# onesamblack/distributed-torch-horovod-gcp

Hardware: NVIDIA H100
Metric: images/sec (whole job, device-timed, max over ranks) ResNet-50 synthetic ImageNet training (higher is better)
Workload: dtype bf16

## Files before the change

distributed_torch_horovod_gcp_b200/csrc/conv_sm90.cu:

```cuda
#include <cuda.h>
#include <cuda_bf16.h>
#include <cuda_runtime.h>
#include <limits.h>
#include <stdint.h>
#include <stdio.h>
#include <stdlib.h>
#include <string.h>

#include "sm90_common.cuh"

namespace {

constexpr int MAX_TAPS = 9;
constexpr int MAX_CLASSES = 4;

struct ConvTap {
  int amap;
  int dw, dh;
  int wcol;
};
struct ConvClass {
  int ntaps;
  int out_map;
  ConvTap taps[MAX_TAPS];
};
struct ConvParams {
  GemmParams g;
  int num_classes;
  int kc_per_tap;
  int bw, bh, bn;
  int sw, sh;
  int tiles_w, tiles_h, tiles_n;
  int num_taps_total;
  int out_w, out_h, out_n;
  ConvClass cls[MAX_CLASSES];
};
struct alignas(64) ConvMaps {
  CUtensorMap a[4];
  CUtensorMap b;
  CUtensorMap out[4];
};

enum { MODE_FPROP = 0, MODE_DGRAD = 1, MODE_WGRAD = 2 };

template <int BN, int MODE>
struct ConvWork {
  static constexpr bool kStats = MODE == MODE_FPROP, kSplitK = MODE == MODE_WGRAD;
  static constexpr bool B_MN = MODE != MODE_FPROP;
  const ConvMaps& maps;
  const ConvParams& p;
  int nnb, pix_tiles, tiles, items, kb_per_split;

  __device__ ConvWork(const ConvMaps& maps_, const ConvParams& p_)
      : maps(maps_), p(p_), nnb(p_.g.num_n_blocks), pix_tiles(p_.tiles_w * p_.tiles_h * p_.tiles_n),
        tiles(MODE == MODE_WGRAD ? p_.g.num_m_blocks * nnb * p_.num_taps_total : p_.num_classes * pix_tiles * nnb),
        items(tiles * p_.g.splits),
        kb_per_split(MODE == MODE_WGRAD ? (pix_tiles + p_.g.splits - 1) / p_.g.splits : 0) {}
  __device__ void prefetch() const {
    for (int i = 0; i < 4; ++i) tma_prefetch_desc(&maps.a[i]);
    tma_prefetch_desc(&maps.b);
    for (int i = 0; i < 4; ++i) tma_prefetch_desc(&maps.out[i]);
  }
  __device__ int num_kb(int w) const {
    if (MODE != MODE_WGRAD) return p.cls[(w / nnb) / pix_tiles].ntaps * p.kc_per_tap;
    const int kb0 = (w / tiles) * kb_per_split;
    return min(kb0 + kb_per_split, pix_tiles) - kb0;
  }
  template <class Next>
  __device__ void load(int w, Next& next) const {
    if (MODE != MODE_WGRAD) {
      const int nt = w % nnb;
      const int rest = w / nnb;
      const int mt = rest % pix_tiles;
      const ConvClass& cl = p.cls[rest / pix_tiles];
      const int w0 = (mt % p.tiles_w) * p.bw;
      const int h0 = ((mt / p.tiles_w) % p.tiles_h) * p.bh;
      const int n0 = (mt / (p.tiles_w * p.tiles_h)) * p.bn;
      const int n_idx = nt * BN;
      for (int t = 0; t < cl.ntaps; ++t) {
        const ConvTap tap = cl.taps[t];
        for (int kc = 0; kc < p.kc_per_tap; ++kc) {
          const Stage s = next();
          tma_load_4d(&maps.a[tap.amap], s.bar, s.a, kc * BLOCK_K, w0 + tap.dw, h0 + tap.dh, n0);
          if (!B_MN) {
            tma_load_2d(&maps.b, s.bar, s.b, tap.wcol + kc * BLOCK_K, n_idx);
          } else {
#pragma unroll
            for (int c = 0; c < BN / 64; ++c)
              tma_load_2d(&maps.b, s.bar, s.b + c * (BLOCK_K * 128), tap.wcol + n_idx + 64 * c, kc * BLOCK_K);
          }
        }
      }
    } else {
      const int tile = w % tiles, split = w / tiles;
      const ConvTap tap = p.cls[0].taps[tile % p.num_taps_total];
      const int mn = tile / p.num_taps_total;
      const int m_idx = (mn / nnb) * BLOCK_M;
      const int n_idx = (mn % nnb) * BN;
      const int kb0 = split * kb_per_split;
      const int kb1 = min(kb0 + kb_per_split, pix_tiles);
      for (int kb = kb0; kb < kb1; ++kb) {
        const int w0 = (kb % p.tiles_w) * p.bw;
        const int h0 = ((kb / p.tiles_w) % p.tiles_h) * p.bh;
        const int n0 = (kb / (p.tiles_w * p.tiles_h)) * p.bn;
        const Stage s = next();
#pragma unroll
        for (int c = 0; c < BLOCK_M / 64; ++c)
          tma_load_4d(&maps.out[0], s.bar, s.a + c * (BLOCK_K * 128), m_idx + 64 * c, w0, h0, n0);
#pragma unroll
        for (int c = 0; c < BN / 64; ++c)
          tma_load_4d(&maps.a[tap.amap], s.bar, s.b + c * (BLOCK_K * 128), n_idx + 64 * c, w0 + tap.dw,
                      h0 + tap.dh, n0);
      }
    }
  }
  __device__ Slab slab(int w, int q) const {
    if (MODE != MODE_WGRAD) {
      const int nt = w % nnb;
      const int rest = w / nnb;
      const int mt = rest % pix_tiles;
      const int r0 = q * 32;
      StoreAt at;
      at.rank4 = 1;
      at.w = (mt % p.tiles_w) * p.bw + (r0 % p.bw);
      at.h = ((mt / p.tiles_w) % p.tiles_h) * p.bh + (r0 / p.bw) % p.bh;
      at.n = (mt / (p.tiles_w * p.tiles_h)) * p.bn + r0 / (p.bw * p.bh);
      at.c_ptr = nullptr;
      at.sw = p.sw; at.sh = p.sh;
      at.vw = p.out_w - at.w; at.vh = p.out_h - at.h; at.vn = p.out_n - at.n;
      return Slab{&maps.out[p.cls[rest / pix_tiles].out_map], nullptr, 0, nt * BN, at, 0, 0, 0};
    }
    const int tile = w % tiles;
    const ConvTap tap = p.cls[0].taps[tile % p.num_taps_total];
    const int mn = tile / p.num_taps_total;
    const int m_idx = (mn / nnb) * BLOCK_M;
    float* c_ptr = (p.g.splits > 1 ? p.g.splitk_ws + (long long)(w / tiles) * p.g.splitk_slice
                                   : reinterpret_cast<float*>(p.g.C)) + tap.wcol;
    return Slab{nullptr, nullptr, m_idx + q * 32, (mn % nnb) * BN, StoreAt{0, 0, 0, 0, c_ptr, 32, 1, 32, 1, 1},
                tile, m_idx, tap.wcol};
  }
};

template <int BN, int MODE>
__global__ void __launch_bounds__(NUM_THREADS, 1)
conv_bf16_kernel(const __grid_constant__ ConvMaps maps, const __grid_constant__ ConvParams p) {
  persistent_body<BN, MODE == MODE_WGRAD, MODE != MODE_FPROP>(ConvWork<BN, MODE>(maps, p), p.g);
}

int make_map4(CUtensorMap* m, const void* ptr, uint64_t C, uint64_t Wd, uint64_t Hd, uint64_t Nd, uint64_t pw,
              uint64_t ph, uint64_t pn, uint32_t bw, uint32_t bh, uint32_t bn) {
  const cuuint64_t dims[4] = {C, Wd, Hd, Nd};
  const cuuint64_t strides[3] = {pw * 2, ph * 2, pn * 2};
  const cuuint32_t box[4] = {64, bw, bh, bn};
  return encode_map(m, ptr, 4, dims, strides, box);
}

void choose_box(int W, int H, int N, int rows, int* bw, int* bh, int* bn) {
  double best = 1e30;
  *bw = 1; *bh = 1; *bn = rows;
  for (int w = 1; w <= rows; w <<= 1) {
    for (int h = 1; w * h <= rows; h <<= 1) {
      const int n = rows / (w * h);
      const double covered = (double)((W + w - 1) / w * w) * ((H + h - 1) / h * h) * ((N + n - 1) / n * n);
      const double score = covered - 1e-3 * w - 1e-6 * h;
      if (score < best) { best = score; *bw = w; *bh = h; *bn = n; }
    }
  }
}

int floordiv2(int e) { return (e >= 0) ? e / 2 : -((-e + 1) / 2); }

struct ConvShape {
  int N, H, W, Cin, Cout, R, S, stride, pad, OH, OW;
};

int check_shape(ConvShape& s) {
  if (s.R != s.S || (s.R != 1 && s.R != 3)) return fail("only 1x1 and 3x3 filters");
  if (s.pad != (s.R - 1) / 2) return fail("padding must be (R-1)/2");
  if (s.stride != 1 && s.stride != 2) return fail("stride must be 1 or 2");
  if (s.stride == 2 && ((s.H | s.W) & 1)) return fail("stride 2 needs even H and W");
  if ((s.Cin % 8) || (s.Cout % 8)) return fail("channels must be multiples of 8");
  s.OH = s.H / s.stride;
  s.OW = s.W / s.stride;
  return 0;
}

int make_parity_maps(CUtensorMap* maps, const void* base, int C, int W, int H, int N, int bw, int bh, int bn) {
  for (int ph = 0; ph < 2; ++ph)
    for (int pw = 0; pw < 2; ++pw) {
      const __nv_bfloat16* ptr = reinterpret_cast<const __nv_bfloat16*>(base) + ((size_t)ph * W + pw) * C;
      if (make_map4(&maps[ph * 2 + pw], ptr, C, W / 2, H / 2, N, 2 * (uint64_t)C, 2 * (uint64_t)W * C,
                    (uint64_t)H * W * C, bw, bh, bn))
        return -1;
    }
  return 0;
}

void forward_taps(ConvClass& cl, int R, int S, int Cin, int stride, int pad) {
  for (int r = 0; r < R; ++r)
    for (int c = 0; c < S; ++c) {
      ConvTap& t = cl.taps[cl.ntaps++];
      const int eh = r - pad, ew = c - pad;
      if (stride == 1) {
        t.amap = 0; t.dh = eh; t.dw = ew;
      } else {
        const int ph = eh & 1, pw = ew & 1;
        t.amap = ph * 2 + pw; t.dh = floordiv2(eh - ph); t.dw = floordiv2(ew - pw);
      }
      t.wcol = (r * S + c) * Cin;
    }
}

void slab_box(ConvParams& p) {
  p.sw = p.bw < 32 ? p.bw : 32;
  p.sh = (32 / p.sw) < p.bh ? (32 / p.sw) : p.bh;
}

template <int MODE>
int launch_conv(const ConvMaps& maps, const ConvParams& p, int BN, int work, int max_ctas, cudaStream_t st) {
  if (BN == 64) return launch_persistent<conv_bf16_kernel<64, MODE>, 64>(work, max_ctas, st, maps, p);
  return launch_persistent<conv_bf16_kernel<128, MODE>, 128>(work, max_ctas, st, maps, p);
}

ConvParams conv_params() {
  ConvParams p;
  memset(&p, 0, sizeof(p));
  p.g.M = INT_MAX;
  p.g.splits = 1;
  p.g.alpha = 1.0f;
  return p;
}

}

extern "C" {

const char* b200dp_conv_last_error() { return g_err; }

int b200dp_conv_fprop(const void* x, const void* w, void* y, int N, int H, int W, int Cin, int Cout, int R, int S,
                      int stride, int pad, int block_n, int max_ctas, float* stats, unsigned long long stream) {
  if (ensure_init()) return -1;
  ConvShape s{N, H, W, Cin, Cout, R, S, stride, pad, 0, 0};
  if (check_shape(s)) return -1;
  if (((uintptr_t)x | (uintptr_t)w | (uintptr_t)y) & 15) return fail("pointers must be 16-byte aligned");
  const int BN = pick_bn(Cout, block_n);
  if (BN < 0) return -1;
  ConvMaps maps;
  ConvParams p = conv_params();
  p.g.N = Cout; p.g.ldc = Cout; p.g.C = y; p.g.out_mode = 0;
  p.g.stats = stats;
  if (stats != nullptr && Cout > STATS_MAX_N) return fail("stats: Cout <= 2048 required");
  p.g.num_n_blocks = (Cout + BN - 1) / BN;
  p.g.num_k_blocks = (Cin + BLOCK_K - 1) / BLOCK_K;
  p.kc_per_tap = p.g.num_k_blocks;
  choose_box(s.OW, s.OH, N, BLOCK_M, &p.bw, &p.bh, &p.bn);
  p.tiles_w = (s.OW + p.bw - 1) / p.bw; p.tiles_h = (s.OH + p.bh - 1) / p.bh; p.tiles_n = (N + p.bn - 1) / p.bn;
  p.num_classes = 1;
  p.num_taps_total = R * S;
  p.out_w = s.OW; p.out_h = s.OH; p.out_n = N;
  forward_taps(p.cls[0], R, S, Cin, stride, pad);
  if (stride == 1) {
    if (make_map4(&maps.a[0], x, Cin, W, H, N, Cin, (uint64_t)W * Cin, (uint64_t)H * W * Cin, p.bw, p.bh, p.bn))
      return -1;
    maps.a[1] = maps.a[2] = maps.a[3] = maps.a[0];
  } else if (make_parity_maps(maps.a, x, Cin, W, H, N, p.bw, p.bh, p.bn)) {
    return -1;
  }
  if (make_map2(&maps.b, w, Cout, (uint64_t)R * S * Cin, (uint64_t)R * S * Cin, BN)) return -1;
  slab_box(p);
  if (make_map4(&maps.out[0], y, Cout, s.OW, s.OH, N, Cout, (uint64_t)s.OW * Cout, (uint64_t)s.OH * s.OW * Cout, p.sw,
                p.sh, 32 / (p.sw * p.sh)))
    return -1;
  maps.out[1] = maps.out[2] = maps.out[3] = maps.out[0];
  const int work = p.tiles_w * p.tiles_h * p.tiles_n * p.g.num_n_blocks;
  return launch_conv<MODE_FPROP>(maps, p, BN, work, max_ctas, (cudaStream_t)(uintptr_t)stream);
}

int b200dp_conv_dgrad(const void* dy, const void* w, void* dx, int N, int H, int W, int Cin, int Cout, int R, int S,
                      int stride, int pad, int block_n, int max_ctas, unsigned long long stream) {
  if (ensure_init()) return -1;
  ConvShape s{N, H, W, Cin, Cout, R, S, stride, pad, 0, 0};
  if (check_shape(s)) return -1;
  if (((uintptr_t)dy | (uintptr_t)w | (uintptr_t)dx) & 15) return fail("pointers must be 16-byte aligned");
  cudaStream_t st = (cudaStream_t)(uintptr_t)stream;
  const int BN = pick_bn(Cin, block_n);
  if (BN < 0) return -1;
  ConvMaps maps;
  ConvParams p = conv_params();
  p.g.N = Cin; p.g.ldc = Cin; p.g.C = dx; p.g.out_mode = 0;
  p.g.num_n_blocks = (Cin + BN - 1) / BN;
  p.g.num_k_blocks = (Cout + BLOCK_K - 1) / BLOCK_K;
  p.kc_per_tap = p.g.num_k_blocks;
  choose_box(s.OW, s.OH, N, BLOCK_M, &p.bw, &p.bh, &p.bn);
  p.tiles_w = (s.OW + p.bw - 1) / p.bw; p.tiles_h = (s.OH + p.bh - 1) / p.bh; p.tiles_n = (N + p.bn - 1) / p.bn;
  p.num_taps_total = R * S;
  p.out_w = s.OW; p.out_h = s.OH; p.out_n = N;
  slab_box(p);
  const int sn = 32 / (p.sw * p.sh);
  if (make_map4(&maps.a[0], dy, Cout, s.OW, s.OH, N, Cout, (uint64_t)s.OW * Cout, (uint64_t)s.OH * s.OW * Cout,
                p.bw, p.bh, p.bn))
    return -1;
  maps.a[1] = maps.a[2] = maps.a[3] = maps.a[0];
  if (make_map2(&maps.b, w, Cout, (uint64_t)R * S * Cin, (uint64_t)R * S * Cin, 64)) return -1;
  if (stride == 1) {
    p.num_classes = 1;
    ConvClass& cl = p.cls[0];
    cl.out_map = 0;
    for (int r = 0; r < R; ++r)
      for (int c = 0; c < S; ++c) {
        ConvTap& t = cl.taps[cl.ntaps++];
        t.amap = 0; t.dh = pad - r; t.dw = pad - c; t.wcol = (r * S + c) * Cin;
      }
    if (make_map4(&maps.out[0], dx, Cin, W, H, N, Cin, (uint64_t)W * Cin, (uint64_t)H * W * Cin, p.sw, p.sh, sn))
      return -1;
    maps.out[1] = maps.out[2] = maps.out[3] = maps.out[0];
  } else {
    if (make_parity_maps(maps.out, dx, Cin, W, H, N, p.sw, p.sh, sn)) return -1;
    bool any_empty = false;
    for (int ph = 0; ph < 2; ++ph)
      for (int pw = 0; pw < 2; ++pw) {
        ConvClass cl;
        memset(&cl, 0, sizeof(cl));
        cl.out_map = ph * 2 + pw;
        for (int r = 0; r < R; ++r) {
          if ((ph + pad - r) & 1) continue;
          for (int c = 0; c < S; ++c) {
            if ((pw + pad - c) & 1) continue;
            ConvTap& t = cl.taps[cl.ntaps++];
            t.amap = 0; t.dh = floordiv2(ph + pad - r); t.dw = floordiv2(pw + pad - c); t.wcol = (r * S + c) * Cin;
          }
        }
        if (cl.ntaps == 0) { any_empty = true; continue; }
        p.cls[p.num_classes++] = cl;
      }
    if (any_empty) {
      cudaError_t e = cudaMemsetAsync(dx, 0, (size_t)N * H * W * Cin * 2, st);
      if (e != cudaSuccess) return fail(cudaGetErrorString(e), (int)e);
    }
  }
  const int work = p.num_classes * p.tiles_w * p.tiles_h * p.tiles_n * p.g.num_n_blocks;
  return launch_conv<MODE_DGRAD>(maps, p, BN, work, max_ctas, st);
}

int b200dp_conv_wgrad(const void* dy, const void* x, void* dw_acc, int N, int H, int W, int Cin, int Cout, int R,
                      int S, int stride, int pad, int splits, int block_n, int max_ctas, unsigned long long stream) {
  if (ensure_init()) return -1;
  ConvShape s{N, H, W, Cin, Cout, R, S, stride, pad, 0, 0};
  if (check_shape(s)) return -1;
  if (((uintptr_t)dy | (uintptr_t)x | (uintptr_t)dw_acc) & 15) return fail("pointers must be 16-byte aligned");
  const int BN = pick_bn(Cin, block_n);
  if (BN < 0) return -1;
  ConvMaps maps;
  ConvParams p = conv_params();
  p.g.M = Cout; p.g.N = Cin; p.g.ldc = R * S * Cin; p.g.C = dw_acc; p.g.out_mode = 1;
  p.g.num_m_blocks = (Cout + BLOCK_M - 1) / BLOCK_M;
  p.g.num_n_blocks = (Cin + BN - 1) / BN;
  choose_box(s.OW, s.OH, N, BLOCK_K, &p.bw, &p.bh, &p.bn);
  p.tiles_w = (s.OW + p.bw - 1) / p.bw; p.tiles_h = (s.OH + p.bh - 1) / p.bh; p.tiles_n = (N + p.bn - 1) / p.bn;
  const int kblocks = p.tiles_w * p.tiles_h * p.tiles_n;
  p.num_classes = 1;
  p.num_taps_total = R * S;
  forward_taps(p.cls[0], R, S, Cin, stride, pad);
  const int tiles = p.g.num_m_blocks * p.g.num_n_blocks * R * S;
  if (splits <= 0) {
    splits = g_num_sms / tiles;
    if (splits < 1) splits = 1;
    const int max_splits = kblocks / 8 > 1 ? kblocks / 8 : 1;
    if (splits > max_splits) splits = max_splits;
  }
  p.g.splits = normalize_splits(splits, kblocks);
  if (stride == 1) {
    if (make_map4(&maps.a[0], x, Cin, W, H, N, Cin, (uint64_t)W * Cin, (uint64_t)H * W * Cin, p.bw, p.bh, p.bn))
      return -1;
    maps.a[1] = maps.a[2] = maps.a[3] = maps.a[0];
  } else if (make_parity_maps(maps.a, x, Cin, W, H, N, p.bw, p.bh, p.bn)) {
    return -1;
  }
  if (make_map4(&maps.out[0], dy, Cout, s.OW, s.OH, N, Cout, (uint64_t)s.OW * Cout, (uint64_t)s.OH * s.OW * Cout,
                p.bw, p.bh, p.bn))
    return -1;
  maps.out[1] = maps.out[2] = maps.out[3] = maps.out[0];
  maps.b = maps.out[0];
  cudaStream_t st = (cudaStream_t)(uintptr_t)stream;
  if (p.g.splits > 1) p.g.splitk_slice = (long long)Cout * p.g.ldc;
  return run_splitk(p.g, tiles, st,
                    [&] { return launch_conv<MODE_WGRAD>(maps, p, BN, tiles * p.g.splits, max_ctas, st); });
}

}
```

distributed_torch_horovod_gcp_b200/csrc/gemm_sm90.cu:

```cuda
#include <cuda.h>
#include <cuda_bf16.h>
#include <cuda_runtime.h>
#include <stdint.h>

#include "sm90_common.cuh"

namespace {

template <int BN, bool A_MN, bool B_MN>
struct GemmWork {
  static constexpr bool kStats = true, kSplitK = true;
  const CUtensorMap *a, *b, *c, *z;
  const GemmParams& p;
  int tiles, items, kb_per_split;

  __device__ GemmWork(const CUtensorMap* a_, const CUtensorMap* b_, const CUtensorMap* c_, const CUtensorMap* z_,
                      const GemmParams& p_)
      : a(a_), b(b_), c(c_), z(z_), p(p_), tiles(p_.num_m_blocks * p_.num_n_blocks), items(tiles * p_.splits),
        kb_per_split((p_.num_k_blocks + p_.splits - 1) / p_.splits) {}
  __device__ void prefetch() const {
    tma_prefetch_desc(a);
    tma_prefetch_desc(b);
    if (p.out_mode == 0) tma_prefetch_desc(c);
    if (p.out_mode == 0 && p.preact != nullptr) tma_prefetch_desc(z);
  }
  __device__ int m_idx(int tile) const {
    return (p.n_fastest ? tile / p.num_n_blocks : tile % p.num_m_blocks) * BLOCK_M;
  }
  __device__ int n_idx(int tile) const { return (p.n_fastest ? tile % p.num_n_blocks : tile / p.num_m_blocks) * BN; }
  __device__ int num_kb(int w) const {
    const int kb0 = (w / tiles) * kb_per_split;
    return min(kb0 + kb_per_split, p.num_k_blocks) - kb0;
  }
  template <class Next>
  __device__ void load(int w, Next& next) const {
    const int tile = w % tiles;
    const int m0 = m_idx(tile), n0 = n_idx(tile);
    const int kb0 = (w / tiles) * kb_per_split;
    const int kb1 = min(kb0 + kb_per_split, p.num_k_blocks);
    for (int kb = kb0; kb < kb1; ++kb) {
      const Stage s = next();
      const int k_idx = kb * BLOCK_K;
      if (!A_MN) {
        tma_load_2d(a, s.bar, s.a, k_idx, m0);
      } else {
#pragma unroll
        for (int c = 0; c < BLOCK_M / 64; ++c)
          tma_load_2d(a, s.bar, s.a + c * (BLOCK_K * 128), m0 + 64 * c, k_idx);
      }
      if (!B_MN) {
        tma_load_2d(b, s.bar, s.b, k_idx, n0);
      } else {
#pragma unroll
        for (int c = 0; c < BN / 64; ++c)
          tma_load_2d(b, s.bar, s.b + c * (BLOCK_K * 128), n0 + 64 * c, k_idx);
      }
    }
  }
  __device__ Slab slab(int w, int q) const {
    const int tile = w % tiles, split = w / tiles;
    const int m0 = m_idx(tile);
    return Slab{c, z, m0 + q * 32, n_idx(tile),
                StoreAt{0, 0, 0, 0, p.splits > 1 ? p.splitk_ws + (long long)split * p.splitk_slice : nullptr},
                tile, m0, 0};
  }
};

template <int BN, bool A_MN, bool B_MN>
__global__ void __launch_bounds__(NUM_THREADS, 1)
gemm_bf16_kernel(const __grid_constant__ CUtensorMap map_a, const __grid_constant__ CUtensorMap map_b,
                 const __grid_constant__ CUtensorMap map_c, const __grid_constant__ CUtensorMap map_z,
                 const __grid_constant__ GemmParams p) {
  persistent_body<BN, A_MN, B_MN>(GemmWork<BN, A_MN, B_MN>(&map_a, &map_b, &map_c, &map_z, p), p);
}

int launch_bn(int BN, int a_mn, int b_mn, const CUtensorMap& ma, const CUtensorMap& mb, const CUtensorMap& mc,
              const CUtensorMap& mz, const GemmParams& p, int max_ctas, cudaStream_t st) {
  const int work = p.num_m_blocks * p.num_n_blocks * p.splits;
#define LAUNCH(BNV, AMN, BMN) \
  launch_persistent<gemm_bf16_kernel<BNV, AMN, BMN>, BNV>(work, max_ctas, st, ma, mb, mc, mz, p)
#define DISPATCH(BNV)                                          \
  if (BN == BNV) {                                             \
    if (!a_mn && !b_mn) return LAUNCH(BNV, false, false);      \
    if (!a_mn && b_mn) return LAUNCH(BNV, false, true);        \
    if (a_mn && !b_mn) return LAUNCH(BNV, true, false);        \
    return LAUNCH(BNV, true, true);                            \
  }
  DISPATCH(64)
  DISPATCH(128)
#undef DISPATCH
#undef LAUNCH
  return fail("unreachable");
}

}

extern "C" {

const char* b200dp_gemm_last_error() { return g_err; }

int b200dp_gemm_bf16(const void* A, const void* B, void* C, int M, int N, int K, int lda, int ldb, int ldc,
                     int a_mn, int b_mn, const void* bias_bf16, const void* bias_f32, const void* residual,
                     void* preact, int act, int out_mode, float alpha, int splits, int block_n, int max_ctas,
                     float* stats, const void* res_mask, unsigned long long stream) {
  if (ensure_init()) return -1;
  if (M <= 0 || N <= 0 || K <= 0) return fail("bad shape");
  if ((N % 8) || (lda % 8) || (ldb % 8) || (ldc % 4) || ((out_mode == 0) && (ldc % 8)))
    return fail("alignment: N, lda, ldb, ldc must be multiples of 8");
  if (((uintptr_t)A | (uintptr_t)B | (uintptr_t)C) & 15) return fail("pointers must be 16-byte aligned");
  const int BN = pick_bn(N, block_n);
  if (BN < 0) return -1;
  GemmParams p{};
  p.M = M; p.N = N; p.ldc = ldc;
  p.num_m_blocks = (M + BLOCK_M - 1) / BLOCK_M;
  p.num_n_blocks = (N + BN - 1) / BN;
  p.num_k_blocks = (K + BLOCK_K - 1) / BLOCK_K;
  p.splits = normalize_splits(splits, p.num_k_blocks);
  if (p.splits > 1 && out_mode != 1) return fail("split-K requires out_mode=1 (fp32 accumulate)");
  p.act = act; p.out_mode = out_mode; p.C = C; p.bias = bias_bf16; p.bias_f32 = bias_f32;
  p.residual = residual; p.preact = preact; p.alpha = alpha;
  p.stats = stats;
  p.res_mask = reinterpret_cast<const unsigned char*>(res_mask);
  if (res_mask != nullptr && (residual == nullptr || preact != nullptr || act > 2 || out_mode != 0 || (N % 64) ||
                              ldc != N))
    return fail("res_mask: plain bf16 residual, dense rows and N % 64 == 0 required");
  if (stats != nullptr && (N > STATS_MAX_N || out_mode != 0)) return fail("stats: N <= 2048 and bf16 output required");
  p.n_fastest = ((size_t)N * (size_t)K * 2 <= ((size_t)20 << 20)) ? 1 : 0;
  CUtensorMap ma, mb, mc, mz;
  if (a_mn ? make_map2(&ma, A, K, M, lda, BLOCK_K) : make_map2(&ma, A, M, K, lda, BLOCK_M)) return -1;
  if (b_mn ? make_map2(&mb, B, K, N, ldb, BLOCK_K) : make_map2(&mb, B, N, K, ldb, BN)) return -1;
  if (out_mode == 0) {
    if (make_map2(&mc, C, M, N, ldc, 32)) return -1;
  } else {
    mc = ma;
  }
  if (out_mode == 0 && preact != nullptr) {
    if (make_map2(&mz, preact, M, N, ldc, 32)) return -1;
  } else {
    mz = mc;
  }
  cudaStream_t st = (cudaStream_t)(uintptr_t)stream;
  if (p.splits > 1) p.splitk_slice = (long long)M * ldc;
  return run_splitk(p, p.num_m_blocks * p.num_n_blocks, st,
                    [&] { return launch_bn(BN, a_mn, b_mn, ma, mb, mc, mz, p, max_ctas, st); });
}

}
```

distributed_torch_horovod_gcp_b200/csrc/sm90_common.cuh:

```cuda
#pragma once
#include <cuda.h>
#include <cuda_bf16.h>
#include <cuda_runtime.h>
#include <stdint.h>
#include <stdio.h>

namespace {

constexpr int BLOCK_M = 128;
constexpr int BLOCK_K = 64;
constexpr int WGMMA_K = 16;
constexpr int NUM_THREADS = 384;
constexpr int EPI_WARPS = 8;
constexpr int SMEM_LIMIT = 232448;

struct GemmParams {
  int M, N;
  int ldc;
  int num_m_blocks, num_n_blocks, num_k_blocks;
  int splits;
  int act;
  int out_mode;
  void* C;
  const void* bias;
  const void* bias_f32;
  const void* residual;
  void* preact;
  int n_fastest;
  float alpha;
  const unsigned char* res_mask;
  float* stats;
  float* splitk_ws;
  int* splitk_count;
  long long splitk_slice;
};

constexpr int STATS_MAX_N = 2048;
constexpr int STATS_WARP_FLOATS = 256;
constexpr int STATS_SMEM_BYTES = 8 * STATS_WARP_FLOATS * 4;

__device__ __forceinline__ uint32_t smem_u32(const void* p) {
  return static_cast<uint32_t>(__cvta_generic_to_shared(p));
}
__device__ __forceinline__ void mbar_init(uint64_t* bar, uint32_t count) {
  asm volatile("mbarrier.init.shared::cta.b64 [%0], %1;" ::"r"(smem_u32(bar)), "r"(count));
}
__device__ __forceinline__ void mbar_expect_tx(uint64_t* bar, uint32_t bytes) {
  asm volatile("mbarrier.arrive.expect_tx.shared::cta.b64 _, [%0], %1;" ::"r"(smem_u32(bar)),
               "r"(bytes)
               : "memory");
}
__device__ __forceinline__ void mbar_arrive(uint64_t* bar) {
  asm volatile("mbarrier.arrive.shared::cta.b64 _, [%0];" ::"r"(smem_u32(bar)) : "memory");
}
__device__ __forceinline__ void mbar_wait(uint64_t* bar, uint32_t parity) {
  uint32_t done = 0;
  unsigned long long t0 = 0;
  for (uint32_t tries = 0; !done; ++tries) {
    asm volatile(
        "{\n\t"
        ".reg .pred p;\n\t"
        "mbarrier.try_wait.parity.shared::cta.b64 p, [%1], %2;\n\t"
        "selp.u32 %0, 1, 0, p;\n\t"
        "}\n"
        : "=r"(done)
        : "r"(smem_u32(bar)), "r"(parity)
        : "memory");
    if (!done && (tries & 1023u) == 1023u) {
      unsigned long long now;
      asm volatile("mov.u64 %0, %%globaltimer;" : "=l"(now));
      if (t0 == 0) t0 = now;
      else if (now - t0 > 4000000000ull) __trap();
    }
  }
}
__device__ __forceinline__ void tma_load_2d(const CUtensorMap* map, uint64_t* bar, void* dst, int c0,
                                            int c1) {
  asm volatile(
      "cp.async.bulk.tensor.2d.shared::cluster.global.mbarrier::complete_tx::bytes [%0], [%1, {%3, %4}], "
      "[%2];" ::"r"(smem_u32(dst)),
      "l"(map), "r"(smem_u32(bar)), "r"(c0), "r"(c1)
      : "memory");
}
__device__ __forceinline__ void tma_store_2d(const CUtensorMap* map, const void* src, int c0, int c1) {
  asm volatile("cp.async.bulk.tensor.2d.global.shared::cta.bulk_group [%0, {%2, %3}], [%1];" ::"l"(map),
               "r"(smem_u32(src)), "r"(c0), "r"(c1)
               : "memory");
}
__device__ __forceinline__ void tma_load_4d(const CUtensorMap* map, uint64_t* bar, void* dst, int c0, int c1,
                                            int c2, int c3) {
  asm volatile(
      "cp.async.bulk.tensor.4d.shared::cluster.global.mbarrier::complete_tx::bytes [%0], "
      "[%1, {%3, %4, %5, %6}], [%2];" ::"r"(smem_u32(dst)),
      "l"(map), "r"(smem_u32(bar)), "r"(c0), "r"(c1), "r"(c2), "r"(c3)
      : "memory");
}
__device__ __forceinline__ void tma_store_4d(const CUtensorMap* map, const void* src, int c0, int c1, int c2,
                                             int c3) {
  asm volatile("cp.async.bulk.tensor.4d.global.shared::cta.bulk_group [%0, {%2, %3, %4, %5}], [%1];" ::"l"(map),
               "r"(smem_u32(src)), "r"(c0), "r"(c1), "r"(c2), "r"(c3)
               : "memory");
}
__device__ __forceinline__ void tma_store_commit() { asm volatile("cp.async.bulk.commit_group;" ::: "memory"); }
template <int N>
__device__ __forceinline__ void tma_store_wait_read() {
  asm volatile("cp.async.bulk.wait_group.read %0;" ::"n"(N) : "memory");
}
__device__ __forceinline__ void tma_store_wait_all() { asm volatile("cp.async.bulk.wait_group 0;" ::: "memory"); }
__device__ __forceinline__ void fence_async_smem() { asm volatile("fence.proxy.async.shared::cta;" ::: "memory"); }
__device__ __forceinline__ void tma_prefetch_desc(const CUtensorMap* map) {
  asm volatile("prefetch.tensormap [%0];" ::"l"(map) : "memory");
}
__device__ __forceinline__ void wg_fence() { asm volatile("wgmma.fence.sync.aligned;" ::: "memory"); }
__device__ __forceinline__ void wg_commit() { asm volatile("wgmma.commit_group.sync.aligned;" ::: "memory"); }
template <int N>
__device__ __forceinline__ void wg_wait() {
  asm volatile("wgmma.wait_group.sync.aligned %0;" ::"n"(N) : "memory");
}
template <int R>
__device__ __forceinline__ void wg_fence_operands(float* d) {
#pragma unroll
  for (int i = 0; i < R; ++i) asm volatile("" : "+f"(d[i])::"memory");
}
__device__ __forceinline__ void named_bar(int id, int count) {
  asm volatile("bar.sync %0, %1;" ::"r"(id), "r"(count) : "memory");
}

template <int TA, int TB>
__device__ __forceinline__ void wgmma_bf16_n64(float* d, uint64_t a, uint64_t b, uint32_t acc) {
  asm volatile(
      "{\n\t.reg .pred p;\n\tsetp.ne.b32 p, %34, 0;\n\t"
      "wgmma.mma_async.sync.aligned.m64n64k16.f32.bf16.bf16 {%0, %1, %2, %3, %4, %5, %6, %7, %8, %9, %10, %11, %12, %13, %14, %15, %16, %17, %18, %19, %20, %21, %22, %23, %24, %25, %26, %27, %28, %29, %30, %31}, %32, %33, p, 1, 1, %35, %36;\n\t}\n"
      : "+f"(d[0]), "+f"(d[1]), "+f"(d[2]), "+f"(d[3]), "+f"(d[4]), "+f"(d[5]), "+f"(d[6]), "+f"(d[7]), "+f"(d[8]), "+f"(d[9]), "+f"(d[10]), "+f"(d[11]), "+f"(d[12]), "+f"(d[13]), "+f"(d[14]), "+f"(d[15]), "+f"(d[16]), "+f"(d[17]), "+f"(d[18]), "+f"(d[19]), "+f"(d[20]), "+f"(d[21]), "+f"(d[22]), "+f"(d[23]), "+f"(d[24]), "+f"(d[25]), "+f"(d[26]), "+f"(d[27]), "+f"(d[28]), "+f"(d[29]), "+f"(d[30]), "+f"(d[31])
      : "l"(a), "l"(b), "r"(acc), "n"(TA), "n"(TB));
}

template <int TA, int TB>
__device__ __forceinline__ void wgmma_bf16_n128(float* d, uint64_t a, uint64_t b, uint32_t acc) {
  asm volatile(
      "{\n\t.reg .pred p;\n\tsetp.ne.b32 p, %66, 0;\n\t"
      "wgmma.mma_async.sync.aligned.m64n128k16.f32.bf16.bf16 {%0, %1, %2, %3, %4, %5, %6, %7, %8, %9, %10, %11, %12, %13, %14, %15, %16, %17, %18, %19, %20, %21, %22, %23, %24, %25, %26, %27, %28, %29, %30, %31, %32, %33, %34, %35, %36, %37, %38, %39, %40, %41, %42, %43, %44, %45, %46, %47, %48, %49, %50, %51, %52, %53, %54, %55, %56, %57, %58, %59, %60, %61, %62, %63}, %64, %65, p, 1, 1, %67, %68;\n\t}\n"
      : "+f"(d[0]), "+f"(d[1]), "+f"(d[2]), "+f"(d[3]), "+f"(d[4]), "+f"(d[5]), "+f"(d[6]), "+f"(d[7]), "+f"(d[8]), "+f"(d[9]), "+f"(d[10]), "+f"(d[11]), "+f"(d[12]), "+f"(d[13]), "+f"(d[14]), "+f"(d[15]), "+f"(d[16]), "+f"(d[17]), "+f"(d[18]), "+f"(d[19]), "+f"(d[20]), "+f"(d[21]), "+f"(d[22]), "+f"(d[23]), "+f"(d[24]), "+f"(d[25]), "+f"(d[26]), "+f"(d[27]), "+f"(d[28]), "+f"(d[29]), "+f"(d[30]), "+f"(d[31]), "+f"(d[32]), "+f"(d[33]), "+f"(d[34]), "+f"(d[35]), "+f"(d[36]), "+f"(d[37]), "+f"(d[38]), "+f"(d[39]), "+f"(d[40]), "+f"(d[41]), "+f"(d[42]), "+f"(d[43]), "+f"(d[44]), "+f"(d[45]), "+f"(d[46]), "+f"(d[47]), "+f"(d[48]), "+f"(d[49]), "+f"(d[50]), "+f"(d[51]), "+f"(d[52]), "+f"(d[53]), "+f"(d[54]), "+f"(d[55]), "+f"(d[56]), "+f"(d[57]), "+f"(d[58]), "+f"(d[59]), "+f"(d[60]), "+f"(d[61]), "+f"(d[62]), "+f"(d[63])
      : "l"(a), "l"(b), "r"(acc), "n"(TA), "n"(TB));
}

__device__ __forceinline__ void wgmma_tf32_n32(float* d, uint64_t a, uint64_t b, uint32_t acc) {
  asm volatile(
      "{\n\t.reg .pred p;\n\tsetp.ne.b32 p, %18, 0;\n\t"
      "wgmma.mma_async.sync.aligned.m64n32k8.f32.tf32.tf32 {%0, %1, %2, %3, %4, %5, %6, %7, %8, %9, %10, %11, %12, %13, %14, %15}, %16, %17, p, 1, 1;\n\t}\n"
      : "+f"(d[0]), "+f"(d[1]), "+f"(d[2]), "+f"(d[3]), "+f"(d[4]), "+f"(d[5]), "+f"(d[6]), "+f"(d[7]), "+f"(d[8]), "+f"(d[9]), "+f"(d[10]), "+f"(d[11]), "+f"(d[12]), "+f"(d[13]), "+f"(d[14]), "+f"(d[15])
      : "l"(a), "l"(b), "r"(acc));
}


template <int N>
__device__ __forceinline__ void acc_to_smem(const float* d, uint32_t img, int ld, int row0) {
  const int t = threadIdx.x & 127;
  const int r = row0 + (t >> 5) * 16 + ((t & 31) >> 2);
  const uint32_t p0 = img + (uint32_t)((r * ld + 2 * (t & 3)) * 4);
  const uint32_t p1 = p0 + (uint32_t)(8 * ld * 4);
#pragma unroll
  for (int j = 0; j < N / 8; ++j) {
    asm volatile("st.shared.v2.f32 [%0], {%1, %2};" ::"r"(p0 + j * 32), "f"(d[4 * j]), "f"(d[4 * j + 1]) : "memory");
    asm volatile("st.shared.v2.f32 [%0], {%1, %2};" ::"r"(p1 + j * 32), "f"(d[4 * j + 2]), "f"(d[4 * j + 3]) : "memory");
  }
}
__device__ __forceinline__ void acc_ld32(uint32_t addr, uint32_t* r) {
#pragma unroll
  for (int i = 0; i < 8; ++i)
    asm volatile("ld.shared.v4.b32 {%0, %1, %2, %3}, [%4];"
                 : "=r"(r[4 * i]), "=r"(r[4 * i + 1]), "=r"(r[4 * i + 2]), "=r"(r[4 * i + 3])
                 : "r"(addr + 16 * i)
                 : "memory");
}

__device__ __forceinline__ uint64_t make_desc(uint32_t smem_addr, uint32_t lbo_bytes,
                                              uint32_t sbo_bytes) {
  uint64_t d = 0;
  d |= (uint64_t)((smem_addr & 0x3FFFF) >> 4);
  d |= (uint64_t)((lbo_bytes >> 4) & 0x3FFF) << 16;
  d |= (uint64_t)((sbo_bytes >> 4) & 0x3FFF) << 32;
  d |= (uint64_t)1 << 62;
  return d;
}

__device__ __forceinline__ bool elect_one() {
  uint32_t pred;
  asm volatile(
      "{\n\t"
      ".reg .pred p;\n\t"
      "elect.sync _|p, 0xffffffff;\n\t"
      "selp.u32 %0, 1, 0, p;\n\t"
      "}\n"
      : "=r"(pred));
  return pred != 0;
}

__device__ __forceinline__ uint64_t make_desc_base(uint32_t lbo_bytes, uint32_t sbo_bytes) {
  return make_desc(0, lbo_bytes, sbo_bytes);
}
__device__ __forceinline__ uint64_t desc_addr(uint32_t smem_addr) { return (uint64_t)((smem_addr & 0x3FFFF) >> 4); }

template <int BN, bool TA, bool TB>
__device__ __forceinline__ void wgmma_bf16(float* d, uint64_t a, uint64_t b, uint32_t acc) {
  static_assert(BN == 64 || BN == 128, "wgmma width");
  if constexpr (BN == 64) wgmma_bf16_n64<TA ? 1 : 0, TB ? 1 : 0>(d, a, b, acc);
  else wgmma_bf16_n128<TA ? 1 : 0, TB ? 1 : 0>(d, a, b, acc);
}

template <int BN, bool A_MN, bool B_MN, int STAGES, int A_BYTES, int B_BYTES>
__device__ __forceinline__ void wg_mainloop(float* d, uint32_t sa, uint32_t sb, uint64_t* full_bar, uint64_t* empty_bar,
                                            int& stage, uint32_t& phase, int nkb, int wg) {
  constexpr uint32_t KSTEP_A = A_MN ? ((WGMMA_K * 128) >> 4) : ((WGMMA_K * 2) >> 4);
  constexpr uint32_t KSTEP_B = B_MN ? ((WGMMA_K * 128) >> 4) : ((WGMMA_K * 2) >> 4);
  const uint64_t a0 = (A_MN ? make_desc_base(BLOCK_K * 128, 1024) : make_desc_base(16, 1024)) +
                      desc_addr(sa + (uint32_t)wg * 8192u);
  const uint64_t b0 = (B_MN ? make_desc_base(BLOCK_K * 128, 1024) : make_desc_base(16, 1024)) + desc_addr(sb);
  const bool leader = (threadIdx.x & 127) == 0;
  int prev = -1;
  for (int kb = 0; kb < nkb; ++kb) {
    mbar_wait(&full_bar[stage], phase);
    const uint64_t da = a0 + (uint64_t)(stage * (A_BYTES >> 4));
    const uint64_t db = b0 + (uint64_t)(stage * (B_BYTES >> 4));
    wg_fence();
#pragma unroll
    for (int k = 0; k < BLOCK_K / WGMMA_K; ++k)
      wgmma_bf16<BN, A_MN, B_MN>(d, da + k * KSTEP_A, db + k * KSTEP_B, (kb | k) ? 1u : 0u);
    wg_commit();
    wg_wait<1>();
    if (prev >= 0 && leader) mbar_arrive(&empty_bar[prev]);
    prev = stage;
    if (++stage == STAGES) { stage = 0; phase ^= 1; }
  }
  wg_wait<0>();
  wg_fence_operands<BN / 2>(d);
  if (prev >= 0 && leader) mbar_arrive(&empty_bar[prev]);
}

__device__ __forceinline__ float fast_erf(float x) {
  const float ax = fabsf(x);
  const float t = __fdividef(1.0f, fmaf(0.3275911f, ax, 1.0f));
  float poly = fmaf(1.061405429f, t, -1.453152027f);
  poly = fmaf(poly, t, 1.421413741f);
  poly = fmaf(poly, t, -0.284496736f);
  poly = fmaf(poly, t, 0.254829592f);
  const float y = 1.0f - poly * t * __expf(-ax * ax);
  return copysignf(y, x);
}
__device__ __forceinline__ float gelu_erf(float x) {
  return 0.5f * x * (1.0f + fast_erf(x * 0.70710678118654752f));
}

__device__ __forceinline__ float gelu_erf_grad(float x) {
  const float cdf = 0.5f * (1.0f + fast_erf(x * 0.70710678118654752f));
  const float pdf = 0.3989422804014327f * __expf(-0.5f * x * x);
  return cdf + x * pdf;
}

__device__ __forceinline__ void unpack8(const uint4& x, float* f) {
  const uint32_t wv[4] = {x.x, x.y, x.z, x.w};
#pragma unroll
  for (int t = 0; t < 4; ++t) {
    f[2 * t] = __uint_as_float(wv[t] << 16);
    f[2 * t + 1] = __uint_as_float(wv[t] & 0xffff0000u);
  }
}

__device__ __forceinline__ uint4 pack8(const float* v) {
  uint32_t wv[4];
#pragma unroll
  for (int t = 0; t < 4; ++t) {
    __nv_bfloat162 h = __floats2bfloat162_rn(v[2 * t], v[2 * t + 1]);
    wv[t] = *reinterpret_cast<uint32_t*>(&h);
  }
  return make_uint4(wv[0], wv[1], wv[2], wv[3]);
}

template <int BN>
struct Cfg {
  static constexpr int A_BYTES = BLOCK_M * BLOCK_K * 2;
  static constexpr int B_BYTES = BN * BLOCK_K * 2;
  static constexpr int STAGE_BYTES = A_BYTES + B_BYTES;
  static constexpr int ACC_LD = BN + 4;
  static constexpr int ACC_BYTES = BLOCK_M * ACC_LD * 4;
  static constexpr int STORE_BYTES = EPI_WARPS * 2 * 4096;
  static constexpr int FIXED_BYTES = STORE_BYTES + ACC_BYTES + 1024  + 256  + STATS_SMEM_BYTES;
  static constexpr int STAGES = (SMEM_LIMIT - FIXED_BYTES) / STAGE_BYTES > 4 ? 4 : (SMEM_LIMIT - FIXED_BYTES) / STAGE_BYTES;
  static constexpr int SMEM_BYTES = STAGES * STAGE_BYTES + FIXED_BYTES;
  static_assert(STAGES >= 2, "shared memory");
};

struct StoreAt {
  int rank4, w, h, n;
  void* c_ptr;
  int sw, sh, vw, vh, vn;
};

__device__ __forceinline__ void epi_sts128(uint32_t addr, const uint4& v) {
  asm volatile("st.shared.v4.b32 [%0], {%1, %2, %3, %4};" ::"r"(addr), "r"(v.x), "r"(v.y), "r"(v.z), "r"(v.w) : "memory");
}
__device__ __forceinline__ uint4 epi_lds128(uint32_t addr) {
  uint4 v;
  asm volatile("ld.shared.v4.b32 {%0, %1, %2, %3}, [%4];" : "=r"(v.x), "=r"(v.y), "=r"(v.z), "=r"(v.w) : "r"(addr) : "memory");
  return v;
}
__device__ __forceinline__ uint32_t prmt_sign(uint32_t a, uint32_t sel) {
  uint32_t d;
  asm("prmt.b32 %0, %1, %2, %3;" : "=r"(d) : "r"(a), "r"(0u), "r"(sel));
  return d;
}
__device__ __forceinline__ uint4 pack8r(const uint32_t* r) {
  uint4 o;
  asm("cvt.rn.bf16x2.f32 %0, %1, %2;" : "=r"(o.x) : "f"(__uint_as_float(r[1])), "f"(__uint_as_float(r[0])));
  asm("cvt.rn.bf16x2.f32 %0, %1, %2;" : "=r"(o.y) : "f"(__uint_as_float(r[3])), "f"(__uint_as_float(r[2])));
  asm("cvt.rn.bf16x2.f32 %0, %1, %2;" : "=r"(o.z) : "f"(__uint_as_float(r[5])), "f"(__uint_as_float(r[4])));
  asm("cvt.rn.bf16x2.f32 %0, %1, %2;" : "=r"(o.w) : "f"(__uint_as_float(r[7])), "f"(__uint_as_float(r[6])));
  return o;
}

template <int BN>
__device__ __forceinline__ void epilogue_rows(const GemmParams& p, const CUtensorMap* map_c,
                                              const CUtensorMap* map_z, uint32_t acc_img, int acc, int q,
                                              int lane, int m_row0, int n_idx, int c_begin, int c_end,
                                              uint8_t* my_store, const StoreAt at, float* s_stats) {
  const int row = m_row0 + lane;
  const bool row_ok = row < p.M;
  const bool to_tma = p.out_mode == 0;
  const bool z_tma = p.preact != nullptr && to_tma;
  const bool res_smem = p.residual != nullptr && p.preact == nullptr && p.out_mode != 1;
  const bool plain = to_tma && p.alpha == 1.0f && p.bias == nullptr && p.bias_f32 == nullptr &&
                     p.preact == nullptr && p.act == 0 && p.residual == nullptr;
  const bool res_only = to_tma && res_smem && p.alpha == 1.0f && p.bias == nullptr && p.bias_f32 == nullptr &&
                        p.act == 0;
  const uint32_t store_s = smem_u32(my_store);
  const uint32_t lane_row = (uint32_t)lane * 128u;
  const uint32_t lsw = (uint32_t)(lane & 7);
#pragma unroll 1
  for (int c0 = c_begin; c0 < c_end; c0 += 64) {
    const int col0 = n_idx + c0;
    if (col0 >= p.N) continue;
    const int ncols = min(64, p.N - col0);
    uint4 resv[8];
    if (res_smem) {
      const __nv_bfloat16* rbase = reinterpret_cast<const __nv_bfloat16*>(p.residual);
#pragma unroll
      for (int i = 0; i < 8; ++i) {
        const int rr = i * 4 + (lane >> 3), u = lane & 7;
        resv[i] = (m_row0 + rr < p.M && u * 8 < ncols)
                      ? *reinterpret_cast<const uint4*>(rbase + (size_t)(m_row0 + rr) * p.ldc + col0 + u * 8)
                      : make_uint4(0, 0, 0, 0);
      }
      if (p.res_mask != nullptr) {
        uint32_t mbits[8];
#pragma unroll
        for (int i = 0; i < 8; ++i) {
          const int rr = i * 4 + (lane >> 3), u = lane & 7;
          mbits[i] = (m_row0 + rr < p.M && u * 8 < ncols)
                         ? (uint32_t)p.res_mask[(size_t)(m_row0 + rr) * (size_t)(p.N >> 3) + (size_t)((col0 >> 3) + u)]
                         : 0u;
        }
#pragma unroll
        for (int i = 0; i < 8; ++i) {
          const uint32_t rep = mbits[i] * 0x01010101u;
          const uint32_t lo = (rep & 0x08040201u) + 0x7f7f7f7fu, hi = (rep & 0x80402010u) + 0x7f7f7f7fu;
          resv[i].x &= prmt_sign(lo, 0x9988u);
          resv[i].y &= prmt_sign(lo, 0xbbaau);
          resv[i].z &= prmt_sign(hi, 0x9988u);
          resv[i].w &= prmt_sign(hi, 0xbbaau);
        }
      }
    }
    const bool dbuf = to_tma && !z_tma && !res_smem;
    const int par = (((c0 - c_begin) >> 6) + acc * (((c_end - c_begin) >> 6) & 1)) & 1;
    const uint32_t out_s = store_s + ((dbuf && par) ? 4096u : 0u);
    if (res_smem) {
      if (lane == 0) tma_store_wait_read<0>();
      __syncwarp();
#pragma unroll
      for (int i = 0; i < 8; ++i) {
        const int rr = i * 4 + (lane >> 3), u = lane & 7;
        epi_sts128(store_s + 4096u + rr * 128 + ((u ^ (rr & 7)) << 4), resv[i]);
      }
      __syncwarp();
    }
    const uint32_t taddr = acc_img + (uint32_t)(((q * 32 + lane) * (BN + 4) + c0) * 4);
    if (plain) {
      uint32_t r[32];
      acc_ld32(taddr, r);
      if (lane == 0) {
        if (dbuf) tma_store_wait_read<1>();
        else tma_store_wait_read<0>();
      }
      __syncwarp();
#pragma unroll
      for (int j = 0; j < 4; ++j) epi_sts128(out_s + lane_row + ((j ^ lsw) << 4), pack8r(r + j * 8));
      if (ncols > 32) {
        acc_ld32(taddr + 128, r);
#pragma unroll
        for (int j = 0; j < 4; ++j) epi_sts128(out_s + lane_row + (((4 + j) ^ lsw) << 4), pack8r(r + j * 8));
      }
    } else if (res_only) {
#pragma unroll 1
      for (int half = 0; half < 2; ++half) {
        if (half * 32 >= ncols) break;
        uint32_t r[32];
        acc_ld32(taddr + half * 128, r);
#pragma unroll
        for (int j = 0; j < 4; ++j) {
          const uint32_t off = lane_row + (((half * 4 + j) ^ lsw) << 4);
          const uint4 rv = epi_lds128(store_s + 4096u + off);
          const uint32_t rw[4] = {rv.x, rv.y, rv.z, rv.w};
          uint4 o;
          uint32_t* ow = reinterpret_cast<uint32_t*>(&o);
#pragma unroll
          for (int w = 0; w < 4; ++w) {
            const float s0 = __uint_as_float(r[j * 8 + 2 * w]) + __uint_as_float(rw[w] << 16);
            const float s1 = __uint_as_float(r[j * 8 + 2 * w + 1]) + __uint_as_float(rw[w] & 0xffff0000u);
            asm("cvt.rn.bf16x2.f32 %0, %1, %2;" : "=r"(ow[w]) : "f"(s1), "f"(s0));
          }
          epi_sts128(out_s + off, o);
        }
      }
    } else {
#pragma unroll 1
    for (int half = 0; half < 2; ++half) {
      const int hc = half * 32;
      if (hc >= ncols) break;
      const int hcols = min(32, ncols - hc);
      uint32_t r[32];
      acc_ld32(taddr + hc * 4, r);
      float v[32];
#pragma unroll
      for (int i = 0; i < 32; ++i) v[i] = __uint_as_float(r[i]);
      if (p.alpha != 1.0f) {
#pragma unroll
        for (int i = 0; i < 32; ++i) v[i] *= p.alpha;
      }
      if (p.out_mode != 1) {
        if (p.bias != nullptr) {
          const __nv_bfloat16* b = reinterpret_cast<const __nv_bfloat16*>(p.bias) + col0 + hc;
#pragma unroll
          for (int i = 0; i < 32; ++i)
            if (i < hcols) v[i] += __bfloat162float(b[i]);
        } else if (p.bias_f32 != nullptr) {
          const float* b = reinterpret_cast<const float*>(p.bias_f32) + col0 + hc;
#pragma unroll
          for (int i = 0; i < 32; ++i)
            if (i < hcols) v[i] += b[i];
        }
        if (p.preact != nullptr) {
          if (z_tma) {
            if (half == 0) {
              if (lane == 0) tma_store_wait_read<0>();
              __syncwarp();
            }
#pragma unroll
            for (int j = 0; j < 4; ++j)
              epi_sts128(store_s + 4096u + lane_row + (((half * 4 + j) ^ lsw) << 4), pack8(v + j * 8));
          } else if (row_ok) {
            uint4* pp = reinterpret_cast<uint4*>(reinterpret_cast<__nv_bfloat16*>(p.preact) +
                                                 (size_t)row * p.ldc + col0 + hc);
#pragma unroll
            for (int j = 0; j < 4; ++j)
              if (j * 8 < hcols) pp[j] = pack8(v + j * 8);
          }
        }
        if (p.act == 1) {
#pragma unroll
          for (int i = 0; i < 32; ++i) v[i] = fmaxf(v[i], 0.0f);
        } else if (p.act == 2) {
#pragma unroll
          for (int i = 0; i < 32; ++i) v[i] = gelu_erf(v[i]);
        }
        if (p.residual != nullptr && (row_ok || res_smem)) {
          const uint4* rp = reinterpret_cast<const uint4*>(
              reinterpret_cast<const __nv_bfloat16*>(p.residual) + (size_t)row * p.ldc + col0 + hc);
#pragma unroll
          for (int j = 0; j < 4; ++j) {
            if (j * 8 < hcols) {
              float a[8];
              unpack8(res_smem ? epi_lds128(store_s + 4096u + lane_row + (((half * 4 + j) ^ lsw) << 4)) : rp[j], a);
#pragma unroll
              for (int t = 0; t < 8; ++t) {
                if (p.act == 3) v[j * 8 + t] *= gelu_erf_grad(a[t]);
                else if (p.act == 4) v[j * 8 + t] = a[t] > 0.0f ? v[j * 8 + t] : 0.0f;
                else v[j * 8 + t] += a[t];
              }
            }
          }
        }
      }
      if (to_tma) {
        if (half == 0) {
          if (lane == 0) {
            if (dbuf) tma_store_wait_read<1>();
            else tma_store_wait_read<0>();
          }
          __syncwarp();
        }
#pragma unroll
        for (int j = 0; j < 4; ++j)
          epi_sts128(out_s + lane_row + (((half * 4 + j) ^ lsw) << 4), pack8(v + j * 8));
      } else if (p.out_mode == 1) {
        __syncwarp();
#pragma unroll
        for (int j = 0; j < 8; ++j)
          epi_sts128(store_s + lane_row + ((j ^ lsw) << 4),
                 make_uint4(__float_as_uint(v[4 * j]), __float_as_uint(v[4 * j + 1]), __float_as_uint(v[4 * j + 2]),
                            __float_as_uint(v[4 * j + 3])));
        __syncwarp();
        float* cbase = reinterpret_cast<float*>(at.c_ptr ? at.c_ptr : p.C);
        const int ch = lane & 7;
#pragma unroll
        for (int it = 0; it < 8; ++it) {
          const int rr = it * 4 + (lane >> 3);
          const uint4 t = epi_lds128(store_s + rr * 128 + ((ch ^ (rr & 7)) << 4));
          if (m_row0 + rr < p.M && ch * 4 < hcols) {
            float* dst = cbase + (size_t)(m_row0 + rr) * p.ldc + col0 + hc + ch * 4;
            if (p.splits > 1)
              asm volatile("st.global.v4.b32 [%0], {%1, %2, %3, %4};" ::"l"(dst), "r"(t.x), "r"(t.y), "r"(t.z),
                           "r"(t.w)
                           : "memory");
            else
              asm volatile("red.global.add.v4.f32 [%0], {%1, %2, %3, %4};" ::"l"(dst), "r"(t.x), "r"(t.y), "r"(t.z),
                           "r"(t.w)
                           : "memory");
          }
        }
        __syncwarp();
      } else if (row_ok) {
        float* dst = reinterpret_cast<float*>(at.c_ptr ? at.c_ptr : p.C) + (size_t)row * p.ldc + col0 + hc;
#pragma unroll
        for (int j = 0; j < 8; ++j)
          if (j * 4 < hcols)
            reinterpret_cast<float4*>(dst)[j] = make_float4(v[4 * j], v[4 * j + 1], v[4 * j + 2], v[4 * j + 3]);
      }
    }
    }
    if (to_tma) {
      fence_async_smem();
      __syncwarp();
      if (s_stats != nullptr) {
        float sum_lo = 0.f, sum_hi = 0.f, sq_lo = 0.f, sq_hi = 0.f;
        const uint32_t base = out_s + (uint32_t)((lane & 3) << 2);
        const uint32_t u = (uint32_t)(lane >> 2);
        if (at.rank4 || m_row0 + 32 > p.M) {
          bool ok;
          if (at.rank4) {
            const int rw = lane % at.sw, rh = (lane / at.sw) % at.sh, rn = lane / (at.sw * at.sh);
            ok = rw < at.vw && rh < at.vh && rn < at.vn;
          } else {
            ok = m_row0 + lane < p.M;
          }
          const uint32_t rows_ok = __ballot_sync(0xffffffffu, ok);
#pragma unroll
          for (int rr = 0; rr < 32; ++rr) {
            uint32_t w;
            asm volatile("ld.shared.u32 %0, [%1];" : "=r"(w) : "r"(base + rr * 128 + ((u ^ (rr & 7)) << 4)));
            if (!((rows_ok >> rr) & 1u)) w = 0u;
            const float lo = __uint_as_float(w << 16), hi = __uint_as_float(w & 0xffff0000u);
            sum_lo += lo; sum_hi += hi;
            sq_lo = fmaf(lo, lo, sq_lo); sq_hi = fmaf(hi, hi, sq_hi);
          }
        } else {
#pragma unroll
          for (int rr = 0; rr < 32; ++rr) {
            uint32_t w;
            asm volatile("ld.shared.u32 %0, [%1];" : "=r"(w) : "r"(base + rr * 128 + ((u ^ (rr & 7)) << 4)));
            const float lo = __uint_as_float(w << 16), hi = __uint_as_float(w & 0xffff0000u);
            sum_lo += lo; sum_hi += hi;
            sq_lo = fmaf(lo, lo, sq_lo); sq_hi = fmaf(hi, hi, sq_hi);
          }
        }
        const uint32_t ps = smem_u32(s_stats) + (uint32_t)(((c0 - c_begin) + 2 * lane) << 2);
        float a0, a1, b0, b1;
        asm volatile("ld.shared.v2.f32 {%0, %1}, [%2];" : "=f"(a0), "=f"(a1) : "r"(ps));
        asm volatile("ld.shared.v2.f32 {%0, %1}, [%2];" : "=f"(b0), "=f"(b1) : "r"(ps + (STATS_WARP_FLOATS / 2) * 4));
        asm volatile("st.shared.v2.f32 [%0], {%1, %2};" ::"r"(ps), "f"(a0 + sum_lo), "f"(a1 + sum_hi) : "memory");
        asm volatile("st.shared.v2.f32 [%0], {%1, %2};" ::"r"(ps + (STATS_WARP_FLOATS / 2) * 4), "f"(b0 + sq_lo),
                     "f"(b1 + sq_hi)
                     : "memory");
      }
      if (lane == 0) {
        const uint8_t* buf = my_store + (out_s - store_s);
        if (at.rank4) {
          tma_store_4d(map_c, buf, col0, at.w, at.h, at.n);
        } else {
          tma_store_2d(map_c, buf, col0, m_row0);
          if (p.preact != nullptr) tma_store_2d(map_z, buf + 4096, col0, m_row0);
        }
        tma_store_commit();
      }
    }
  }
}

constexpr int STATS_MAX_CTAS = 256;
__device__ float g_stats_slots[STATS_MAX_CTAS * 2 * STATS_MAX_N];
__device__ unsigned int g_stats_done;
__device__ __forceinline__ float* stats_slot() { return g_stats_slots + (size_t)blockIdx.x * (2 * STATS_MAX_N); }
__device__ __forceinline__ void stats_zero(float* s_stats, int nthreads, int N) {
  for (int i = threadIdx.x; i < 8 * STATS_WARP_FLOATS; i += nthreads) s_stats[i] = 0.f;
  float* slot = stats_slot();
  for (int i = threadIdx.x; i < N; i += nthreads) {
    slot[i] = 0.f;
    slot[STATS_MAX_N + i] = 0.f;
  }
}
__device__ __forceinline__ void stats_finalize(const GemmParams& p, int epi_tid) {
  __shared__ bool last;
  __threadfence();
  asm volatile("bar.sync 2, 256;" ::: "memory");
  if (epi_tid == 0) last = atomicAdd(&g_stats_done, 1u) == gridDim.x - 1;
  asm volatile("bar.sync 2, 256;" ::: "memory");
  if (!last) return;
  __threadfence();
  for (int c = epi_tid; c < p.N; c += 256) {
    float s = 0.f, q = 0.f;
    for (unsigned b = 0; b < gridDim.x; ++b) {
      s += __ldcg(g_stats_slots + (size_t)b * (2 * STATS_MAX_N) + c);
      q += __ldcg(g_stats_slots + (size_t)b * (2 * STATS_MAX_N) + STATS_MAX_N + c);
    }
    p.stats[c] += s;
    p.stats[p.N + c] += q;
  }
  if (epi_tid == 0) g_stats_done = 0u;
}

__device__ __forceinline__ void splitk_finish_tile(const GemmParams& p, int tile, int m_idx, int n_idx, int bn,
                                                   long long c_off, int epi_tid, int* s_last) {
  __threadfence();
  asm volatile("bar.sync 3, 256;" ::: "memory");
  if (epi_tid == 0) *s_last = atomicAdd(p.splitk_count + tile, 1) == p.splits - 1;
  asm volatile("bar.sync 3, 256;" ::: "memory");
  if (!*s_last) return;
  __threadfence();
  const int rows = min(BLOCK_M, p.M - m_idx), c4n = min(bn, p.N - n_idx) >> 2;
  float* C = reinterpret_cast<float*>(p.C);
  for (int e = epi_tid; e < rows * c4n; e += 256) {
    const long long off = c_off + (long long)(m_idx + e / c4n) * p.ldc + n_idx + (e % c4n) * 4;
    float4 s = __ldcg(reinterpret_cast<const float4*>(p.splitk_ws + off));
    for (int k = 1; k < p.splits; ++k) {
      const float4 v = __ldcg(reinterpret_cast<const float4*>(p.splitk_ws + (long long)k * p.splitk_slice + off));
      s.x += v.x; s.y += v.y; s.z += v.z; s.w += v.w;
    }
    float4* c = reinterpret_cast<float4*>(C + off);
    float4 o = *c;
    o.x += s.x; o.y += s.y; o.z += s.z; o.w += s.w;
    *c = o;
  }
}

template <int BN>
__device__ __forceinline__ void stats_flush(const GemmParams& p, float* s_stats, int n_idx, int epi_tid) {
  constexpr int HALF = (BN >= 128) ? BN / 2 : BN;
  asm volatile("bar.sync 2, 256;" ::: "memory");
  if (epi_tid < BN) {
    const int h = epi_tid / HALF, l = epi_tid % HALF;
    const float* r = s_stats + (h * 4) * STATS_WARP_FLOATS + l;
    float s = 0.f, q = 0.f;
#pragma unroll
    for (int k = 0; k < 4; ++k) {
      s += r[k * STATS_WARP_FLOATS];
      q += r[k * STATS_WARP_FLOATS + STATS_WARP_FLOATS / 2];
    }
    if (n_idx + epi_tid < p.N) {
      float* slot = stats_slot();
      slot[n_idx + epi_tid] += s;
      slot[STATS_MAX_N + n_idx + epi_tid] += q;
    }
  }
  asm volatile("bar.sync 2, 256;" ::: "memory");
#pragma unroll
  for (int i = 0; i < 8; ++i) s_stats[i * 256 + epi_tid] = 0.f;
  asm volatile("bar.sync 2, 256;" ::: "memory");
}

struct Stage {
  uint8_t* a;
  uint8_t* b;
  uint64_t* bar;
};
struct Slab {
  const CUtensorMap* map_c;
  const CUtensorMap* map_z;
  int m_row0, n_idx;
  StoreAt at;
  int tile, m_idx;
  long long c_off;
};

template <int BN, bool A_MN, bool B_MN, class Work>
__device__ __forceinline__ void persistent_body(const Work& wk, const GemmParams& p) {
  using C = Cfg<BN>;
  extern __shared__ __align__(1024) uint8_t smem_raw[];
  uint8_t* smem = reinterpret_cast<uint8_t*>((reinterpret_cast<uintptr_t>(smem_raw) + 1023) &
                                             ~static_cast<uintptr_t>(1023));
  uint8_t* smem_a = smem;
  uint8_t* smem_b = smem + C::STAGES * C::A_BYTES;
  uint8_t* smem_store = smem + C::STAGES * C::STAGE_BYTES;
  uint8_t* smem_acc = smem_store + C::STORE_BYTES;
  uint64_t* bars = reinterpret_cast<uint64_t*>(smem_acc + C::ACC_BYTES);
  uint64_t* full_bar = bars;
  uint64_t* empty_bar = bars + C::STAGES;
  float* s_stats = reinterpret_cast<float*>(reinterpret_cast<uint8_t*>(bars) + 256);
  const bool want_stats = Work::kStats && p.stats != nullptr && p.out_mode == 0;
  if (want_stats) stats_zero(s_stats, NUM_THREADS, p.N);

  const int warp = threadIdx.x >> 5;
  const int lane = threadIdx.x & 31;

  if (warp == 0 && lane == 0) {
    wk.prefetch();
    for (int i = 0; i < C::STAGES; ++i) {
      mbar_init(&full_bar[i], 1);
      mbar_init(&empty_bar[i], 2);
    }
    asm volatile("fence.mbarrier_init.release.cluster;" ::: "memory");
  }
  __syncthreads();

  if (warp < 4) {
    if (warp == 0 && lane == 0) {
      int stage = 0;
      uint32_t phase = 0;
      auto next = [&]() {
        mbar_wait(&empty_bar[stage], phase ^ 1);
        mbar_expect_tx(&full_bar[stage], C::STAGE_BYTES);
        const Stage s{smem_a + stage * C::A_BYTES, smem_b + stage * C::B_BYTES, &full_bar[stage]};
        if (++stage == C::STAGES) { stage = 0; phase ^= 1; }
        return s;
      };
      for (int w = blockIdx.x; w < wk.items; w += gridDim.x) wk.load(w, next);
    }
  } else {
    const int cw = warp - 4;
    const int wg = cw >> 2;
    const int q = cw & 3;
    const int half = cw >> 2;
    const int c_begin = (BN >= 128) ? half * (BN / 2) : 0;
    const int c_end = (BN >= 128) ? c_begin + BN / 2 : (half == 0 ? BN : 0);
    const int epi_tid = cw * 32 + lane;
    uint8_t* my_store = smem_store + cw * (2 * 4096);
    float* my_stats = s_stats + cw * STATS_WARP_FLOATS;
    const uint32_t img = smem_u32(smem_acc);
    __shared__ int s_last;
    int stats_n = -1;
    int stage = 0, acc = 0;
    uint32_t phase = 0;
    float d[BN / 2];
    for (int w = blockIdx.x; w < wk.items; w += gridDim.x) {
      const Slab s = wk.slab(w, q);
      wg_mainloop<BN, A_MN, B_MN, C::STAGES, C::A_BYTES, C::B_BYTES>(d, smem_u32(smem_a), smem_u32(smem_b), full_bar,
                                                                     empty_bar, stage, phase, wk.num_kb(w), wg);
      if (want_stats && s.n_idx != stats_n) {
        if (stats_n >= 0) stats_flush<BN>(p, s_stats, stats_n, epi_tid);
        stats_n = s.n_idx;
      }
      named_bar(1, 256);
      acc_to_smem<BN>(d, img, BN + 4, wg * 64);
      named_bar(1, 256);
      epilogue_rows<BN>(p, s.map_c, s.map_z, img, acc, q, lane, s.m_row0, s.n_idx, c_begin, c_end, my_store, s.at,
                        want_stats ? my_stats : nullptr);
      if (Work::kSplitK && p.splits > 1) {
        const Slab t = wk.slab(w, q);
        splitk_finish_tile(p, t.tile, t.m_idx, t.n_idx, BN, t.c_off, epi_tid, &s_last);
      }
      acc ^= 1;
    }
    if (want_stats && stats_n >= 0) stats_flush<BN>(p, s_stats, stats_n, epi_tid);
    if (want_stats) stats_finalize(p, epi_tid);
    if (p.out_mode == 0 && lane == 0) tma_store_wait_all();
  }
}

typedef CUresult (*EncodeTiledFn)(CUtensorMap*, CUtensorMapDataType, cuuint32_t, void*, const cuuint64_t*,
                                  const cuuint64_t*, const cuuint32_t*, const cuuint32_t*,
                                  CUtensorMapInterleave, CUtensorMapSwizzle, CUtensorMapL2promotion,
                                  CUtensorMapFloatOOBfill);
EncodeTiledFn g_encode = nullptr;
thread_local char g_err[512];
int g_num_sms = 0;

int fail(const char* msg, int code = 0) {
  snprintf(g_err, sizeof(g_err), "%s (%d)", msg, code);
  return -1;
}

inline void bind_primary_context() {
  static thread_local bool bound = false;
  if (!bound) {
    cudaFree(nullptr);
    bound = true;
  }
}

int ensure_init() {
  bind_primary_context();
  if (g_encode) return 0;
  void* fn = nullptr;
  cudaDriverEntryPointQueryResult st;
  cudaError_t e = cudaGetDriverEntryPoint("cuTensorMapEncodeTiled", &fn, cudaEnableDefault, &st);
  if (e != cudaSuccess || st != cudaDriverEntryPointSuccess || !fn)
    return fail("cuTensorMapEncodeTiled entry point unavailable", (int)e);
  g_encode = reinterpret_cast<EncodeTiledFn>(fn);
  int dev = 0;
  cudaGetDevice(&dev);
  cudaDeviceGetAttribute(&g_num_sms, cudaDevAttrMultiProcessorCount, dev);
  return 0;
}

int encode_map(CUtensorMap* m, const void* ptr, int rank, const cuuint64_t* dims, const cuuint64_t* byte_strides,
               const cuuint32_t* box) {
  const cuuint32_t estr[4] = {1, 1, 1, 1};
  CUresult r = g_encode(m, CU_TENSOR_MAP_DATA_TYPE_BFLOAT16, rank, const_cast<void*>(ptr), dims, byte_strides, box,
                        estr, CU_TENSOR_MAP_INTERLEAVE_NONE, CU_TENSOR_MAP_SWIZZLE_128B,
                        CU_TENSOR_MAP_L2_PROMOTION_L2_256B, CU_TENSOR_MAP_FLOAT_OOB_FILL_NONE);
  if (r != CUDA_SUCCESS) return fail("cuTensorMapEncodeTiled failed", (int)r);
  return 0;
}

int make_map2(CUtensorMap* m, const void* ptr, uint64_t rows, uint64_t cols, uint64_t ld, uint32_t box_rows) {
  const cuuint64_t dims[2] = {cols, rows};
  const cuuint64_t strides[1] = {ld * 2};
  const cuuint32_t box[2] = {64, box_rows};
  return encode_map(m, ptr, 2, dims, strides, box);
}

template <auto Kernel>
int smem_attr_once(int bytes) {
  static bool attr_set = false;
  if (!attr_set) {
    cudaError_t e = cudaFuncSetAttribute(Kernel, cudaFuncAttributeMaxDynamicSharedMemorySize, bytes);
    if (e != cudaSuccess) return fail(cudaGetErrorString(e), (int)e);
    attr_set = true;
  }
  return 0;
}

template <auto Kernel, int BN, class... Args>
int launch_persistent(int work, int max_ctas, cudaStream_t st, const Args&... args) {
  if (smem_attr_once<Kernel>(Cfg<BN>::SMEM_BYTES)) return -1;
  int grid = work < g_num_sms ? work : g_num_sms;
  if (max_ctas > 0 && grid > max_ctas) grid = max_ctas;
  if (grid > STATS_MAX_CTAS) grid = STATS_MAX_CTAS;
  Kernel<<<grid, NUM_THREADS, Cfg<BN>::SMEM_BYTES, st>>>(args...);
  cudaError_t e = cudaGetLastError();
  if (e != cudaSuccess) return fail(cudaGetErrorString(e), (int)e);
  return 0;
}

template <class Launch>
int run_splitk(GemmParams& p, int tiles, cudaStream_t st, Launch&& launch) {
  void* ws = nullptr;
  if (p.splits > 1) {
    const size_t slices = (size_t)p.splits * (size_t)p.splitk_slice * sizeof(float);
    cudaError_t e = cudaMallocAsync(&ws, slices + (size_t)tiles * sizeof(int), st);
    if (e == cudaSuccess) {
      p.splitk_ws = reinterpret_cast<float*>(ws);
      p.splitk_count = reinterpret_cast<int*>(reinterpret_cast<char*>(ws) + slices);
      e = cudaMemsetAsync(p.splitk_count, 0, (size_t)tiles * sizeof(int), st);
    }
    if (e != cudaSuccess) return fail(cudaGetErrorString(e), (int)e);
  }
  const int rc = launch();
  if (ws != nullptr) {
    cudaError_t e = cudaFreeAsync(ws, st);
    if (e != cudaSuccess && rc == 0) return fail(cudaGetErrorString(e), (int)e);
  }
  return rc;
}

int normalize_splits(int splits, int kblocks) {
  if (splits > kblocks) splits = kblocks;
  if (splits < 1) splits = 1;
  const int per = (kblocks + splits - 1) / splits;
  return (kblocks + per - 1) / per;
}

int pick_bn(int n, int block_n) {
  if (block_n == 0) return n > 64 ? 128 : 64;
  if (block_n == 256) return 128;
  if (block_n != 64 && block_n != 128) return fail("block_n must be 64/128/256");
  return block_n;
}

}
```

Before: 4744.

## Write epilogue directly from WGMMA fragments into swizzled bf16 staging tile

Replaces the fp32 accumulator round-trip through shared memory with a direct fragment-to-bf16 write into a single swizzled staging tile that TMA then stores. Residual is loaded from global into registers before the barrier and staged in place. The preact (z) output moves from a TMA store to per-thread global stores. The freed shared memory allows more pipeline stages, and setmaxnreg rebalances registers between the producer and consumer warpgroups. In exchange, the kernel must now wait for prior TMA store reads before reusing the single staging buffer, and preact writes become uncoalesced.

After: 5694, median of 6. +20.0%, better.

```diff
diff --git a/distributed_torch_horovod_gcp_b200/csrc/conv_sm90.cu b/distributed_torch_horovod_gcp_b200/csrc/conv_sm90.cu
--- a/distributed_torch_horovod_gcp_b200/csrc/conv_sm90.cu
+++ b/distributed_torch_horovod_gcp_b200/csrc/conv_sm90.cu
@@ -128,7 +128,7 @@
       at.c_ptr = nullptr;
       at.sw = p.sw; at.sh = p.sh;
       at.vw = p.out_w - at.w; at.vh = p.out_h - at.h; at.vn = p.out_n - at.n;
-      return Slab{&maps.out[p.cls[rest / pix_tiles].out_map], nullptr, 0, nt * BN, at, 0, 0, 0};
+      return Slab{&maps.out[p.cls[rest / pix_tiles].out_map], 0, nt * BN, at, 0, 0, 0};
     }
     const int tile = w % tiles;
     const ConvTap tap = p.cls[0].taps[tile % p.num_taps_total];
@@ -136,7 +136,7 @@
     const int m_idx = (mn / nnb) * BLOCK_M;
     float* c_ptr = (p.g.splits > 1 ? p.g.splitk_ws + (long long)(w / tiles) * p.g.splitk_slice
                                    : reinterpret_cast<float*>(p.g.C)) + tap.wcol;
-    return Slab{nullptr, nullptr, m_idx + q * 32, (mn % nnb) * BN, StoreAt{0, 0, 0, 0, c_ptr, 32, 1, 32, 1, 1},
+    return Slab{nullptr, m_idx + q * 32, (mn % nnb) * BN, StoreAt{0, 0, 0, 0, c_ptr, 32, 1, 32, 1, 1},
                 tile, m_idx, tap.wcol};
   }
 };
diff --git a/distributed_torch_horovod_gcp_b200/csrc/gemm_sm90.cu b/distributed_torch_horovod_gcp_b200/csrc/gemm_sm90.cu
--- a/distributed_torch_horovod_gcp_b200/csrc/gemm_sm90.cu
+++ b/distributed_torch_horovod_gcp_b200/csrc/gemm_sm90.cu
@@ -10,19 +10,17 @@
 template <int BN, bool A_MN, bool B_MN>
 struct GemmWork {
   static constexpr bool kStats = true, kSplitK = true;
-  const CUtensorMap *a, *b, *c, *z;
+  const CUtensorMap *a, *b, *c;
   const GemmParams& p;
   int tiles, items, kb_per_split;
 
-  __device__ GemmWork(const CUtensorMap* a_, const CUtensorMap* b_, const CUtensorMap* c_, const CUtensorMap* z_,
-                      const GemmParams& p_)
-      : a(a_), b(b_), c(c_), z(z_), p(p_), tiles(p_.num_m_blocks * p_.num_n_blocks), items(tiles * p_.splits),
+  __device__ GemmWork(const CUtensorMap* a_, const CUtensorMap* b_, const CUtensorMap* c_, const GemmParams& p_)
+      : a(a_), b(b_), c(c_), p(p_), tiles(p_.num_m_blocks * p_.num_n_blocks), items(tiles * p_.splits),
         kb_per_split((p_.num_k_blocks + p_.splits - 1) / p_.splits) {}
   __device__ void prefetch() const {
     tma_prefetch_desc(a);
     tma_prefetch_desc(b);
     if (p.out_mode == 0) tma_prefetch_desc(c);
-    if (p.out_mode == 0 && p.preact != nullptr) tma_prefetch_desc(z);
   }
   __device__ int m_idx(int tile) const {
     return (p.n_fastest ? tile / p.num_n_blocks : tile % p.num_m_blocks) * BLOCK_M;
@@ -60,7 +58,7 @@
   __device__ Slab slab(int w, int q) const {
     const int tile = w % tiles, split = w / tiles;
     const int m0 = m_idx(tile);
-    return Slab{c, z, m0 + q * 32, n_idx(tile),
+    return Slab{c, m0 + q * 32, n_idx(tile),
                 StoreAt{0, 0, 0, 0, p.splits > 1 ? p.splitk_ws + (long long)split * p.splitk_slice : nullptr},
                 tile, m0, 0};
   }
@@ -69,16 +67,15 @@
 template <int BN, bool A_MN, bool B_MN>
 __global__ void __launch_bounds__(NUM_THREADS, 1)
 gemm_bf16_kernel(const __grid_constant__ CUtensorMap map_a, const __grid_constant__ CUtensorMap map_b,
-                 const __grid_constant__ CUtensorMap map_c, const __grid_constant__ CUtensorMap map_z,
-                 const __grid_constant__ GemmParams p) {
-  persistent_body<BN, A_MN, B_MN>(GemmWork<BN, A_MN, B_MN>(&map_a, &map_b, &map_c, &map_z, p), p);
+                 const __grid_constant__ CUtensorMap map_c, const __grid_constant__ GemmParams p) {
+  persistent_body<BN, A_MN, B_MN>(GemmWork<BN, A_MN, B_MN>(&map_a, &map_b, &map_c, p), p);
 }
 
 int launch_bn(int BN, int a_mn, int b_mn, const CUtensorMap& ma, const CUtensorMap& mb, const CUtensorMap& mc,
-              const CUtensorMap& mz, const GemmParams& p, int max_ctas, cudaStream_t st) {
+              const GemmParams& p, int max_ctas, cudaStream_t st) {
   const int work = p.num_m_blocks * p.num_n_blocks * p.splits;
 #define LAUNCH(BNV, AMN, BMN) \
-  launch_persistent<gemm_bf16_kernel<BNV, AMN, BMN>, BNV>(work, max_ctas, st, ma, mb, mc, mz, p)
+  launch_persistent<gemm_bf16_kernel<BNV, AMN, BMN>, BNV>(work, max_ctas, st, ma, mb, mc, p)
 #define DISPATCH(BNV)                                          \
   if (BN == BNV) {                                             \
     if (!a_mn && !b_mn) return LAUNCH(BNV, false, false);      \
@@ -126,7 +123,7 @@
     return fail("res_mask: plain bf16 residual, dense rows and N % 64 == 0 required");
   if (stats != nullptr && (N > STATS_MAX_N || out_mode != 0)) return fail("stats: N <= 2048 and bf16 output required");
   p.n_fastest = ((size_t)N * (size_t)K * 2 <= ((size_t)20 << 20)) ? 1 : 0;
-  CUtensorMap ma, mb, mc, mz;
+  CUtensorMap ma, mb, mc;
   if (a_mn ? make_map2(&ma, A, K, M, lda, BLOCK_K) : make_map2(&ma, A, M, K, lda, BLOCK_M)) return -1;
   if (b_mn ? make_map2(&mb, B, K, N, ldb, BLOCK_K) : make_map2(&mb, B, N, K, ldb, BN)) return -1;
   if (out_mode == 0) {
@@ -134,15 +131,10 @@
   } else {
     mc = ma;
   }
-  if (out_mode == 0 && preact != nullptr) {
-    if (make_map2(&mz, preact, M, N, ldc, 32)) return -1;
-  } else {
-    mz = mc;
-  }
   cudaStream_t st = (cudaStream_t)(uintptr_t)stream;
   if (p.splits > 1) p.splitk_slice = (long long)M * ldc;
   return run_splitk(p, p.num_m_blocks * p.num_n_blocks, st,
-                    [&] { return launch_bn(BN, a_mn, b_mn, ma, mb, mc, mz, p, max_ctas, st); });
+                    [&] { return launch_bn(BN, a_mn, b_mn, ma, mb, mc, p, max_ctas, st); });
 }
 
 }
diff --git a/distributed_torch_horovod_gcp_b200/csrc/sm90_common.cuh b/distributed_torch_horovod_gcp_b200/csrc/sm90_common.cuh
--- a/distributed_torch_horovod_gcp_b200/csrc/sm90_common.cuh
+++ b/distributed_torch_horovod_gcp_b200/csrc/sm90_common.cuh
@@ -11,7 +11,6 @@
 constexpr int BLOCK_K = 64;
 constexpr int WGMMA_K = 16;
 constexpr int NUM_THREADS = 384;
-constexpr int EPI_WARPS = 8;
 constexpr int SMEM_LIMIT = 232448;
 
 struct GemmParams {
@@ -153,27 +152,6 @@
 }
 
 
-template <int N>
-__device__ __forceinline__ void acc_to_smem(const float* d, uint32_t img, int ld, int row0) {
-  const int t = threadIdx.x & 127;
-  const int r = row0 + (t >> 5) * 16 + ((t & 31) >> 2);
-  const uint32_t p0 = img + (uint32_t)((r * ld + 2 * (t & 3)) * 4);
-  const uint32_t p1 = p0 + (uint32_t)(8 * ld * 4);
-#pragma unroll
-  for (int j = 0; j < N / 8; ++j) {
-    asm volatile("st.shared.v2.f32 [%0], {%1, %2};" ::"r"(p0 + j * 32), "f"(d[4 * j]), "f"(d[4 * j + 1]) : "memory");
-    asm volatile("st.shared.v2.f32 [%0], {%1, %2};" ::"r"(p1 + j * 32), "f"(d[4 * j + 2]), "f"(d[4 * j + 3]) : "memory");
-  }
-}
-__device__ __forceinline__ void acc_ld32(uint32_t addr, uint32_t* r) {
-#pragma unroll
-  for (int i = 0; i < 8; ++i)
-    asm volatile("ld.shared.v4.b32 {%0, %1, %2, %3}, [%4];"
-                 : "=r"(r[4 * i]), "=r"(r[4 * i + 1]), "=r"(r[4 * i + 2]), "=r"(r[4 * i + 3])
-                 : "r"(addr + 16 * i)
-                 : "memory");
-}
-
 __device__ __forceinline__ uint64_t make_desc(uint32_t smem_addr, uint32_t lbo_bytes,
                                               uint32_t sbo_bytes) {
   uint64_t d = 0;
@@ -266,28 +244,18 @@
   }
 }
 
-__device__ __forceinline__ uint4 pack8(const float* v) {
-  uint32_t wv[4];
-#pragma unroll
-  for (int t = 0; t < 4; ++t) {
-    __nv_bfloat162 h = __floats2bfloat162_rn(v[2 * t], v[2 * t + 1]);
-    wv[t] = *reinterpret_cast<uint32_t*>(&h);
-  }
-  return make_uint4(wv[0], wv[1], wv[2], wv[3]);
-}
-
 template <int BN>
 struct Cfg {
   static constexpr int A_BYTES = BLOCK_M * BLOCK_K * 2;
   static constexpr int B_BYTES = BN * BLOCK_K * 2;
   static constexpr int STAGE_BYTES = A_BYTES + B_BYTES;
-  static constexpr int ACC_LD = BN + 4;
-  static constexpr int ACC_BYTES = BLOCK_M * ACC_LD * 4;
-  static constexpr int STORE_BYTES = EPI_WARPS * 2 * 4096;
-  static constexpr int FIXED_BYTES = STORE_BYTES + ACC_BYTES + 1024  + 256  + STATS_SMEM_BYTES;
-  static constexpr int STAGES = (SMEM_LIMIT - FIXED_BYTES) / STAGE_BYTES > 4 ? 4 : (SMEM_LIMIT - FIXED_BYTES) / STAGE_BYTES;
+  static constexpr int NCH = BN / 64;
+  static constexpr int STORE_BYTES = BLOCK_M * BN * 2;
+  static constexpr int FIXED_BYTES = STORE_BYTES + 1024  + 256  + STATS_SMEM_BYTES;
+  static constexpr int STAGES = (SMEM_LIMIT - FIXED_BYTES) / STAGE_BYTES;
   static constexpr int SMEM_BYTES = STAGES * STAGE_BYTES + FIXED_BYTES;
-  static_assert(STAGES >= 2, "shared memory");
+  static_assert(STAGES >= 4, "shared memory");
+  static_assert(2 * STAGES * 8 <= 256, "barrier space");
 };
 
 struct StoreAt {
@@ -299,9 +267,12 @@
 __device__ __forceinline__ void epi_sts128(uint32_t addr, const uint4& v) {
   asm volatile("st.shared.v4.b32 [%0], {%1, %2, %3, %4};" ::"r"(addr), "r"(v.x), "r"(v.y), "r"(v.z), "r"(v.w) : "memory");
 }
-__device__ __forceinline__ uint4 epi_lds128(uint32_t addr) {
-  uint4 v;
-  asm volatile("ld.shared.v4.b32 {%0, %1, %2, %3}, [%4];" : "=r"(v.x), "=r"(v.y), "=r"(v.z), "=r"(v.w) : "r"(addr) : "memory");
+__device__ __forceinline__ void epi_sts32(uint32_t addr, uint32_t v) {
+  asm volatile("st.shared.b32 [%0], %1;" ::"r"(addr), "r"(v) : "memory");
+}
+__device__ __forceinline__ uint32_t epi_lds32(uint32_t addr) {
+  uint32_t v;
+  asm volatile("ld.shared.b32 %0, [%1];" : "=r"(v) : "r"(addr) : "memory");
   return v;
 }
 __device__ __forceinline__ uint32_t prmt_sign(uint32_t a, uint32_t sel) {
@@ -309,288 +280,204 @@
   asm("prmt.b32 %0, %1, %2, %3;" : "=r"(d) : "r"(a), "r"(0u), "r"(sel));
   return d;
 }
-__device__ __forceinline__ uint4 pack8r(const uint32_t* r) {
-  uint4 o;
-  asm("cvt.rn.bf16x2.f32 %0, %1, %2;" : "=r"(o.x) : "f"(__uint_as_float(r[1])), "f"(__uint_as_float(r[0])));
-  asm("cvt.rn.bf16x2.f32 %0, %1, %2;" : "=r"(o.y) : "f"(__uint_as_float(r[3])), "f"(__uint_as_float(r[2])));
-  asm("cvt.rn.bf16x2.f32 %0, %1, %2;" : "=r"(o.z) : "f"(__uint_as_float(r[5])), "f"(__uint_as_float(r[4])));
-  asm("cvt.rn.bf16x2.f32 %0, %1, %2;" : "=r"(o.w) : "f"(__uint_as_float(r[7])), "f"(__uint_as_float(r[6])));
+__device__ __forceinline__ uint32_t cvt_bf16x2(float lo, float hi) {
+  uint32_t o;
+  asm("cvt.rn.bf16x2.f32 %0, %1, %2;" : "=r"(o) : "f"(hi), "f"(lo));
   return o;
 }
 
 template <int BN>
-__device__ __forceinline__ void epilogue_rows(const GemmParams& p, const CUtensorMap* map_c,
-                                              const CUtensorMap* map_z, uint32_t acc_img, int acc, int q,
-                                              int lane, int m_row0, int n_idx, int c_begin, int c_end,
-                                              uint8_t* my_store, const StoreAt at, float* s_stats) {
-  const int row = m_row0 + lane;
-  const bool row_ok = row < p.M;
-  const bool to_tma = p.out_mode == 0;
-  const bool z_tma = p.preact != nullptr && to_tma;
-  const bool res_smem = p.residual != nullptr && p.preact == nullptr && p.out_mode != 1;
-  const bool plain = to_tma && p.alpha == 1.0f && p.bias == nullptr && p.bias_f32 == nullptr &&
+__device__ __forceinline__ uint32_t stage_off(int r, int u) {
+  return (uint32_t)((((r >> 5) * (BN / 64) + (u >> 3)) << 12) + ((r & 31) << 7) + (((u ^ r) & 7) << 4));
+}
+
+template <int BN>
+__device__ __forceinline__ void res_load(const GemmParams& p, uint4* rv, int m0, int r0, int n_idx, int lane) {
+  const __nv_bfloat16* rbase = reinterpret_cast<const __nv_bfloat16*>(p.residual);
+#pragma unroll
+  for (int i = 0; i < BN / 16; ++i) {
+    const int e = i * 32 + lane, row = m0 + r0 + e / (BN / 8), col = n_idx + (e % (BN / 8)) * 8;
+    rv[i] = (row < p.M && col < p.N) ? *reinterpret_cast<const uint4*>(rbase + (size_t)row * p.ldc + col)
+                                     : make_uint4(0, 0, 0, 0);
+  }
+  if (p.res_mask != nullptr) {
+    uint32_t mbits[BN / 16];
+#pragma unroll
+    for (int i = 0; i < BN / 16; ++i) {
+      const int e = i * 32 + lane, row = m0 + r0 + e / (BN / 8), col = n_idx + (e % (BN / 8)) * 8;
+      mbits[i] = (row < p.M && col < p.N) ? (uint32_t)p.res_mask[(size_t)row * (size_t)(p.N >> 3) + (size_t)(col >> 3)]
+                                          : 0u;
+    }
+#pragma unroll
+    for (int i = 0; i < BN / 16; ++i) {
+      const uint32_t rep = mbits[i] * 0x01010101u;
+      const uint32_t lo = (rep & 0x08040201u) + 0x7f7f7f7fu, hi = (rep & 0x80402010u) + 0x7f7f7f7fu;
+      rv[i].x &= prmt_sign(lo, 0x9988u);
+      rv[i].y &= prmt_sign(lo, 0xbbaau);
+      rv[i].z &= prmt_sign(hi, 0x9988u);
+      rv[i].w &= prmt_sign(hi, 0xbbaau);
+    }
+  }
+}
+template <int BN>
+__device__ __forceinline__ void res_stage(const uint4* rv, uint32_t stg, int r0, int lane) {
+#pragma unroll
+  for (int i = 0; i < BN / 16; ++i) {
+    const int e = i * 32 + lane;
+    epi_sts128(stg + stage_off<BN>(r0 + e / (BN / 8), e % (BN / 8)), rv[i]);
+  }
+}
+
+template <int BN>
+__device__ __forceinline__ void epilogue_frag(const GemmParams& p, const float* d, uint32_t stg, int wg, int m0,
+                                              int n_idx, float* cbase) {
+  const int t = threadIdx.x & 127, lane = t & 31;
+  const int r = wg * 64 + (t >> 5) * 16 + (lane >> 2);
+  const uint32_t x = (uint32_t)(r & 7);
+  const uint32_t sbase = stg + (uint32_t)(((r >> 5) * (BN / 64)) << 12) + (uint32_t)((r & 31) << 7) +
+                         (uint32_t)(lane & 3) * 4u;
+  auto sa = [&](int j, int h) -> uint32_t {
+    return sbase + (uint32_t)(h * 1024 + ((j >> 3) << 12)) + ((((uint32_t)j & 7u) ^ x) << 4);
+  };
+  const bool plain = p.out_mode == 0 && p.alpha == 1.0f && p.bias == nullptr && p.bias_f32 == nullptr &&
                      p.preact == nullptr && p.act == 0 && p.residual == nullptr;
-  const bool res_only = to_tma && res_smem && p.alpha == 1.0f && p.bias == nullptr && p.bias_f32 == nullptr &&
-                        p.act == 0;
-  const uint32_t store_s = smem_u32(my_store);
-  const uint32_t lane_row = (uint32_t)lane * 128u;
-  const uint32_t lsw = (uint32_t)(lane & 7);
+  const bool res_only = p.out_mode == 0 && p.residual != nullptr && p.preact == nullptr && p.alpha == 1.0f &&
+                        p.bias == nullptr && p.bias_f32 == nullptr && p.act == 0;
+  if (plain) {
+#pragma unroll
+    for (int j = 0; j < BN / 8; ++j)
+#pragma unroll
+      for (int h = 0; h < 2; ++h) epi_sts32(sa(j, h), cvt_bf16x2(d[4 * j + 2 * h], d[4 * j + 2 * h + 1]));
+    return;
+  }
+  if (res_only) {
+#pragma unroll
+    for (int j = 0; j < BN / 8; ++j)
+#pragma unroll
+      for (int h = 0; h < 2; ++h) {
+        const uint32_t a = epi_lds32(sa(j, h));
+        epi_sts32(sa(j, h), cvt_bf16x2(d[4 * j + 2 * h] + __uint_as_float(a << 16),
+                                       d[4 * j + 2 * h + 1] + __uint_as_float(a & 0xffff0000u)));
+      }
+    return;
+  }
+  const int cq = n_idx + 2 * (lane & 3);
+#pragma unroll
+  for (int j = 0; j < BN / 8; ++j) {
+    const int col = cq + 8 * j;
+    const bool col_ok = col < p.N;
+#pragma unroll
+    for (int h = 0; h < 2; ++h) {
+      const int row = m0 + r + 8 * h;
+      float v0 = d[4 * j + 2 * h], v1 = d[4 * j + 2 * h + 1];
+      if (p.alpha != 1.0f) {
+        v0 *= p.alpha;
+        v1 *= p.alpha;
+      }
+      if (p.out_mode != 1) {
+        if (p.bias != nullptr) {
+          if (col_ok) {
+            const __nv_bfloat16* b = reinterpret_cast<const __nv_bfloat16*>(p.bias) + col;
+            v0 += __bfloat162float(b[0]);
+            v1 += __bfloat162float(b[1]);
+          }
+        } else if (p.bias_f32 != nullptr) {
+          if (col_ok) {
+            const float* b = reinterpret_cast<const float*>(p.bias_f32) + col;
+            v0 += b[0];
+            v1 += b[1];
+          }
+        }
+        if (p.preact != nullptr && row < p.M && col_ok)
+          *reinterpret_cast<uint32_t*>(reinterpret_cast<__nv_bfloat16*>(p.preact) + (size_t)row * p.ldc + col) =
+              cvt_bf16x2(v0, v1);
+        if (p.act == 1) {
+          v0 = fmaxf(v0, 0.0f);
+          v1 = fmaxf(v1, 0.0f);
+        } else if (p.act == 2) {
+          v0 = gelu_erf(v0);
+          v1 = gelu_erf(v1);
+        }
+        if (p.residual != nullptr) {
+          const uint32_t a = epi_lds32(sa(j, h));
+          const float a0 = __uint_as_float(a << 16), a1 = __uint_as_float(a & 0xffff0000u);
+          if (p.act == 3) {
+            v0 *= gelu_erf_grad(a0);
+            v1 *= gelu_erf_grad(a1);
+          } else if (p.act == 4) {
+            v0 = a0 > 0.0f ? v0 : 0.0f;
+            v1 = a1 > 0.0f ? v1 : 0.0f;
+          } else {
+            v0 += a0;
+            v1 += a1;
+          }
+        }
+      }
+      if (p.out_mode == 0) {
+        epi_sts32(sa(j, h), cvt_bf16x2(v0, v1));
+      } else if (row < p.M && col_ok) {
+        float* dst = cbase + (size_t)row * p.ldc + col;
+        if (p.out_mode == 2 || p.splits > 1)
+          asm volatile("st.global.v2.f32 [%0], {%1, %2};" ::"l"(dst), "f"(v0), "f"(v1) : "memory");
+        else
+          asm volatile("red.global.add.v2.f32 [%0], {%1, %2};" ::"l"(dst), "f"(v0), "f"(v1) : "memory");
+      }
+    }
+  }
+}
+
+template <int BN>
+__device__ __forceinline__ void store_slab(const GemmParams& p, const CUtensorMap* map_c, const uint8_t* stg_ptr,
+                                           int q, int lane, int m_row0, int n_idx, int c_begin, int c_end,
+                                           const StoreAt at, float* s_stats) {
 #pragma unroll 1
   for (int c0 = c_begin; c0 < c_end; c0 += 64) {
     const int col0 = n_idx + c0;
     if (col0 >= p.N) continue;
-    const int ncols = min(64, p.N - col0);
-    uint4 resv[8];
-    if (res_smem) {
-      const __nv_bfloat16* rbase = reinterpret_cast<const __nv_bfloat16*>(p.residual);
-#pragma unroll
-      for (int i = 0; i < 8; ++i) {
-        const int rr = i * 4 + (lane >> 3), u = lane & 7;
-        resv[i] = (m_row0 + rr < p.M && u * 8 < ncols)
-                      ? *reinterpret_cast<const uint4*>(rbase + (size_t)(m_row0 + rr) * p.ldc + col0 + u * 8)
-                      : make_uint4(0, 0, 0, 0);
-      }
-      if (p.res_mask != nullptr) {
-        uint32_t mbits[8];
-#pragma unroll
-        for (int i = 0; i < 8; ++i) {
-          const int rr = i * 4 + (lane >> 3), u = lane & 7;
-          mbits[i] = (m_row0 + rr < p.M && u * 8 < ncols)
-                         ? (uint32_t)p.res_mask[(size_t)(m_row0 + rr) * (size_t)(p.N >> 3) + (size_t)((col0 >> 3) + u)]
-                         : 0u;
+    const uint8_t* buf = stg_ptr + ((q * (BN / 64) + (c0 >> 6)) << 12);
+    if (s_stats != nullptr) {
+      float sum_lo = 0.f, sum_hi = 0.f, sq_lo = 0.f, sq_hi = 0.f;
+      const uint32_t base = smem_u32(buf) + (uint32_t)((lane & 3) << 2);
+      const uint32_t u = (uint32_t)(lane >> 2);
+      if (at.rank4 || m_row0 + 32 > p.M) {
+        bool ok;
+        if (at.rank4) {
+          const int rw = lane % at.sw, rh = (lane / at.sw) % at.sh, rn = lane / (at.sw * at.sh);
+          ok = rw < at.vw && rh < at.vh && rn < at.vn;
+        } else {
+          ok = m_row0 + lane < p.M;
         }
-#pragma unroll
-        for (int i = 0; i < 8; ++i) {
-          const uint32_t rep = mbits[i] * 0x01010101u;
-          const uint32_t lo = (rep & 0x08040201u) + 0x7f7f7f7fu, hi = (rep & 0x80402010u) + 0x7f7f7f7fu;
-          resv[i].x &= prmt_sign(lo, 0x9988u);
-          resv[i].y &= prmt_sign(lo, 0xbbaau);
-          resv[i].z &= prmt_sign(hi, 0x9988u);
-          resv[i].w &= prmt_sign(hi, 0xbbaau);
+        const uint32_t rows_ok = __ballot_sync(0xffffffffu, ok);
+#pragma unroll
+        for (int rr = 0; rr < 32; ++rr) {
+          uint32_t w = epi_lds32(base + rr * 128 + ((u ^ (rr & 7)) << 4));
+          if (!((rows_ok >> rr) & 1u)) w = 0u;
+          const float lo = __uint_as_float(w << 16), hi = __uint_as_float(w & 0xffff0000u);
+          sum_lo += lo; sum_hi += hi;
+          sq_lo = fmaf(lo, lo, sq_lo); sq_hi = fmaf(hi, hi, sq_hi);
         }
-      }
-    }
-    const bool dbuf = to_tma && !z_tma && !res_smem;
-    const int par = (((c0 - c_begin) >> 6) + acc * (((c_end - c_begin) >> 6) & 1)) & 1;
-    const uint32_t out_s = store_s + ((dbuf && par) ? 4096u : 0u);
-    if (res_smem) {
-      if (lane == 0) tma_store_wait_read<0>();
-      __syncwarp();
-#pragma unroll
-      for (int i = 0; i < 8; ++i) {
-        const int rr = i * 4 + (lane >> 3), u = lane & 7;
-        epi_sts128(store_s + 4096u + rr * 128 + ((u ^ (rr & 7)) << 4), resv[i]);
-      }
-      __syncwarp();
-    }
-    const uint32_t taddr = acc_img + (uint32_t)(((q * 32 + lane) * (BN + 4) + c0) * 4);
-    if (plain) {
-      uint32_t r[32];
-      acc_ld32(taddr, r);
-      if (lane == 0) {
-        if (dbuf) tma_store_wait_read<1>();
-        else tma_store_wait_read<0>();
-      }
-      __syncwarp();
-#pragma unroll
-      for (int j = 0; j < 4; ++j) epi_sts128(out_s + lane_row + ((j ^ lsw) << 4), pack8r(r + j * 8));
-      if (ncols > 32) {
-        acc_ld32(taddr + 128, r);
-#pragma unroll
-        for (int j = 0; j < 4; ++j) epi_sts128(out_s + lane_row + (((4 + j) ^ lsw) << 4), pack8r(r + j * 8));
-      }
-    } else if (res_only) {
-#pragma unroll 1
-      for (int half = 0; half < 2; ++half) {
-        if (half * 32 >= ncols) break;
-        uint32_t r[32];
-        acc_ld32(taddr + half * 128, r);
-#pragma unroll
-        for (int j = 0; j < 4; ++j) {
-          const uint32_t off = lane_row + (((half * 4 + j) ^ lsw) << 4);
-          const uint4 rv = epi_lds128(store_s + 4096u + off);
-          const uint32_t rw[4] = {rv.x, rv.y, rv.z, rv.w};
-          uint4 o;
-          uint32_t* ow = reinterpret_cast<uint32_t*>(&o);
-#pragma unroll
-          for (int w = 0; w < 4; ++w) {
-            const float s0 = __uint_as_float(r[j * 8 + 2 * w]) + __uint_as_float(rw[w] << 16);
-            const float s1 = __uint_as_float(r[j * 8 + 2 * w + 1]) + __uint_as_float(rw[w] & 0xffff0000u);
-            asm("cvt.rn.bf16x2.f32 %0, %1, %2;" : "=r"(ow[w]) : "f"(s1), "f"(s0));
-          }
-          epi_sts128(out_s + off, o);
+      } else {
+#pragma unroll
+        for (int rr = 0; rr < 32; ++rr) {
+          const uint32_t w = epi_lds32(base + rr * 128 + ((u ^ (rr & 7)) << 4));
+          const float lo = __uint_as_float(w << 16), hi = __uint_as_float(w & 0xffff0000u);
+          sum_lo += lo; sum_hi += hi;
+          sq_lo = fmaf(lo, lo, sq_lo); sq_hi = fmaf(hi, hi, sq_hi);
         }
       }
-    } else {
-#pragma unroll 1
-    for (int half = 0; half < 2; ++half) {
-      const int hc = half * 32;
-      if (hc >= ncols) break;
-      const int hcols = min(32, ncols - hc);
-      uint32_t r[32];
-      acc_ld32(taddr + hc * 4, r);
-      float v[32];
-#pragma unroll
-      for (int i = 0; i < 32; ++i) v[i] = __uint_as_float(r[i]);
-      if (p.alpha != 1.0f) {
-#pragma unroll
-        for (int i = 0; i < 32; ++i) v[i] *= p.alpha;
-      }
-      if (p.out_mode != 1) {
-        if (p.bias != nullptr) {
-          const __nv_bfloat16* b = reinterpret_cast<const __nv_bfloat16*>(p.bias) + col0 + hc;
-#pragma unroll
-          for (int i = 0; i < 32; ++i)
-            if (i < hcols) v[i] += __bfloat162float(b[i]);
-        } else if (p.bias_f32 != nullptr) {
-          const float* b = reinterpret_cast<const float*>(p.bias_f32) + col0 + hc;
-#pragma unroll
-          for (int i = 0; i < 32; ++i)
-            if (i < hcols) v[i] += b[i];
-        }
-        if (p.preact != nullptr) {
-          if (z_tma) {
-            if (half == 0) {
-              if (lane == 0) tma_store_wait_read<0>();
-              __syncwarp();
-            }
-#pragma unroll
-            for (int j = 0; j < 4; ++j)
-              epi_sts128(store_s + 4096u + lane_row + (((half * 4 + j) ^ lsw) << 4), pack8(v + j * 8));
-          } else if (row_ok) {
-            uint4* pp = reinterpret_cast<uint4*>(reinterpret_cast<__nv_bfloat16*>(p.preact) +
-                                                 (size_t)row * p.ldc + col0 + hc);
-#pragma unroll
-            for (int j = 0; j < 4; ++j)
-              if (j * 8 < hcols) pp[j] = pack8(v + j * 8);
-          }
-        }
-        if (p.act == 1) {
-#pragma unroll
-          for (int i = 0; i < 32; ++i) v[i] = fmaxf(v[i], 0.0f);
-        } else if (p.act == 2) {
-#pragma unroll
-          for (int i = 0; i < 32; ++i) v[i] = gelu_erf(v[i]);
-        }
-        if (p.residual != nullptr && (row_ok || res_smem)) {
-          const uint4* rp = reinterpret_cast<const uint4*>(
-              reinterpret_cast<const __nv_bfloat16*>(p.residual) + (size_t)row * p.ldc + col0 + hc);
-#pragma unroll
-          for (int j = 0; j < 4; ++j) {
-            if (j * 8 < hcols) {
-              float a[8];
-              unpack8(res_smem ? epi_lds128(store_s + 4096u + lane_row + (((half * 4 + j) ^ lsw) << 4)) : rp[j], a);
-#pragma unroll
-              for (int t = 0; t < 8; ++t) {
-                if (p.act == 3) v[j * 8 + t] *= gelu_erf_grad(a[t]);
-                else if (p.act == 4) v[j * 8 + t] = a[t] > 0.0f ? v[j * 8 + t] : 0.0f;
-                else v[j * 8 + t] += a[t];
-              }
-            }
-          }
-        }
-      }
-      if (to_tma) {
-        if (half == 0) {
-          if (lane == 0) {
-            if (dbuf) tma_store_wait_read<1>();
-            else tma_store_wait_read<0>();
-          }
-          __syncwarp();
-        }
-#pragma unroll
-        for (int j = 0; j < 4; ++j)
-          epi_sts128(out_s + lane_row + (((half * 4 + j) ^ lsw) << 4), pack8(v + j * 8));
-      } else if (p.out_mode == 1) {
-        __syncwarp();
-#pragma unroll
-        for (int j = 0; j < 8; ++j)
-          epi_sts128(store_s + lane_row + ((j ^ lsw) << 4),
-                 make_uint4(__float_as_uint(v[4 * j]), __float_as_uint(v[4 * j + 1]), __float_as_uint(v[4 * j + 2]),
-                            __float_as_uint(v[4 * j + 3])));
-        __syncwarp();
-        float* cbase = reinterpret_cast<float*>(at.c_ptr ? at.c_ptr : p.C);
-        const int ch = lane & 7;
-#pragma unroll
-        for (int it = 0; it < 8; ++it) {
-          const int rr = it * 4 + (lane >> 3);
-          const uint4 t = epi_lds128(store_s + rr * 128 + ((ch ^ (rr & 7)) << 4));
-          if (m_row0 + rr < p.M && ch * 4 < hcols) {
-            float* dst = cbase + (size_t)(m_row0 + rr) * p.ldc + col0 + hc + ch * 4;
-            if (p.splits > 1)
-              asm volatile("st.global.v4.b32 [%0], {%1, %2, %3, %4};" ::"l"(dst), "r"(t.x), "r"(t.y), "r"(t.z),
-                           "r"(t.w)
-                           : "memory");
-            else
-              asm volatile("red.global.add.v4.f32 [%0], {%1, %2, %3, %4};" ::"l"(dst), "r"(t.x), "r"(t.y), "r"(t.z),
-                           "r"(t.w)
-                           : "memory");
-          }
-        }
-        __syncwarp();
-      } else if (row_ok) {
-        float* dst = reinterpret_cast<float*>(at.c_ptr ? at.c_ptr : p.C) + (size_t)row * p.ldc + col0 + hc;
-#pragma unroll
-        for (int j = 0; j < 8; ++j)
-          if (j * 4 < hcols)
-            reinterpret_cast<float4*>(dst)[j] = make_float4(v[4 * j], v[4 * j + 1], v[4 * j + 2], v[4 * j + 3]);
-      }
-    }
-    }
-    if (to_tma) {
-      fence_async_smem();
-      __syncwarp();
-      if (s_stats != nullptr) {
-        float sum_lo = 0.f, sum_hi = 0.f, sq_lo = 0.f, sq_hi = 0.f;
-        const uint32_t base = out_s + (uint32_t)((lane & 3) << 2);
-        const uint32_t u = (uint32_t)(lane >> 2);
-        if (at.rank4 || m_row0 + 32 > p.M) {
-          bool ok;
-          if (at.rank4) {
-            const int rw = lane % at.sw, rh = (lane / at.sw) % at.sh, rn = lane / (at.sw * at.sh);
-            ok = rw < at.vw && rh < at.vh && rn < at.vn;
-          } else {
-            ok = m_row0 + lane < p.M;
-          }
-          const uint32_t rows_ok = __ballot_sync(0xffffffffu, ok);
-#pragma unroll
-          for (int rr = 0; rr < 32; ++rr) {
-            uint32_t w;
-            asm volatile("ld.shared.u32 %0, [%1];" : "=r"(w) : "r"(base + rr * 128 + ((u ^ (rr & 7)) << 4)));
-            if (!((rows_ok >> rr) & 1u)) w = 0u;
-            const float lo = __uint_as_float(w << 16), hi = __uint_as_float(w & 0xffff0000u);
-            sum_lo += lo; sum_hi += hi;
-            sq_lo = fmaf(lo, lo, sq_lo); sq_hi = fmaf(hi, hi, sq_hi);
-          }
-        } else {
-#pragma unroll
-          for (int rr = 0; rr < 32; ++rr) {
-            uint32_t w;
-            asm volatile("ld.shared.u32 %0, [%1];" : "=r"(w) : "r"(base + rr * 128 + ((u ^ (rr & 7)) << 4)));
-            const float lo = __uint_as_float(w << 16), hi = __uint_as_float(w & 0xffff0000u);
-            sum_lo += lo; sum_hi += hi;
-            sq_lo = fmaf(lo, lo, sq_lo); sq_hi = fmaf(hi, hi, sq_hi);
-          }
-        }
-        const uint32_t ps = smem_u32(s_stats) + (uint32_t)(((c0 - c_begin) + 2 * lane) << 2);
-        float a0, a1, b0, b1;
-        asm volatile("ld.shared.v2.f32 {%0, %1}, [%2];" : "=f"(a0), "=f"(a1) : "r"(ps));
-        asm volatile("ld.shared.v2.f32 {%0, %1}, [%2];" : "=f"(b0), "=f"(b1) : "r"(ps + (STATS_WARP_FLOATS / 2) * 4));
-        asm volatile("st.shared.v2.f32 [%0], {%1, %2};" ::"r"(ps), "f"(a0 + sum_lo), "f"(a1 + sum_hi) : "memory");
-        asm volatile("st.shared.v2.f32 [%0], {%1, %2};" ::"r"(ps + (STATS_WARP_FLOATS / 2) * 4), "f"(b0 + sq_lo),
-                     "f"(b1 + sq_hi)
-                     : "memory");
-      }
-      if (lane == 0) {
-        const uint8_t* buf = my_store + (out_s - store_s);
-        if (at.rank4) {
-          tma_store_4d(map_c, buf, col0, at.w, at.h, at.n);
-        } else {
-          tma_store_2d(map_c, buf, col0, m_row0);
-          if (p.preact != nullptr) tma_store_2d(map_z, buf + 4096, col0, m_row0);
-        }
-        tma_store_commit();
-      }
+      const uint32_t ps = smem_u32(s_stats) + (uint32_t)(((c0 - c_begin) + 2 * lane) << 2);
+      float a0, a1, b0, b1;
+      asm volatile("ld.shared.v2.f32 {%0, %1}, [%2];" : "=f"(a0), "=f"(a1) : "r"(ps));
+      asm volatile("ld.shared.v2.f32 {%0, %1}, [%2];" : "=f"(b0), "=f"(b1) : "r"(ps + (STATS_WARP_FLOATS / 2) * 4));
+      asm volatile("st.shared.v2.f32 [%0], {%1, %2};" ::"r"(ps), "f"(a0 + sum_lo), "f"(a1 + sum_hi) : "memory");
+      asm volatile("st.shared.v2.f32 [%0], {%1, %2};" ::"r"(ps + (STATS_WARP_FLOATS / 2) * 4), "f"(b0 + sq_lo),
+                   "f"(b1 + sq_hi)
+                   : "memory");
+    }
+    if (lane == 0) {
+      if (at.rank4) tma_store_4d(map_c, buf, col0, at.w, at.h, at.n);
+      else tma_store_2d(map_c, buf, col0, m_row0);
+      tma_store_commit();
     }
   }
 }
@@ -683,10 +570,10 @@
 };
 struct Slab {
   const CUtensorMap* map_c;
-  const CUtensorMap* map_z;
   int m_row0, n_idx;
   StoreAt at;
-  int tile, m_idx;
+  int tile;
+  int m_idx;
   long long c_off;
 };
 
@@ -699,8 +586,7 @@
   uint8_t* smem_a = smem;
   uint8_t* smem_b = smem + C::STAGES * C::A_BYTES;
   uint8_t* smem_store = smem + C::STAGES * C::STAGE_BYTES;
-  uint8_t* smem_acc = smem_store + C::STORE_BYTES;
-  uint64_t* bars = reinterpret_cast<uint64_t*>(smem_acc + C::ACC_BYTES);
+  uint64_t* bars = reinterpret_cast<uint64_t*>(smem_store + C::STORE_BYTES);
   uint64_t* full_bar = bars;
   uint64_t* empty_bar = bars + C::STAGES;
   float* s_stats = reinterpret_cast<float*>(reinterpret_cast<uint8_t*>(bars) + 256);
@@ -721,6 +607,7 @@
   __syncthreads();
 
   if (warp < 4) {
+    asm volatile("setmaxnreg.dec.sync.aligned.u32 40;" ::: "memory");
     if (warp == 0 && lane == 0) {
       int stage = 0;
       uint32_t phase = 0;
@@ -734,19 +621,20 @@
       for (int w = blockIdx.x; w < wk.items; w += gridDim.x) wk.load(w, next);
     }
   } else {
+    asm volatile("setmaxnreg.inc.sync.aligned.u32 232;" ::: "memory");
     const int cw = warp - 4;
     const int wg = cw >> 2;
+    const int r0 = wg * 64 + (cw & 3) * 16;
     const int q = cw & 3;
     const int half = cw >> 2;
     const int c_begin = (BN >= 128) ? half * (BN / 2) : 0;
     const int c_end = (BN >= 128) ? c_begin + BN / 2 : (half == 0 ? BN : 0);
     const int epi_tid = cw * 32 + lane;
-    uint8_t* my_store = smem_store + cw * (2 * 4096);
     float* my_stats = s_stats + cw * STATS_WARP_FLOATS;
-    const uint32_t img = smem_u32(smem_acc);
+    const uint32_t stg = smem_u32(smem_store);
     __shared__ int s_last;
     int stats_n = -1;
-    int stage = 0, acc = 0;
+    int stage = 0;
     uint32_t phase = 0;
     float d[BN / 2];
     for (int w = blockIdx.x; w < wk.items; w += gridDim.x) {
@@ -757,16 +645,26 @@
         if (stats_n >= 0) stats_flush<BN>(p, s_stats, stats_n, epi_tid);
         stats_n = s.n_idx;
       }
-      named_bar(1, 256);
-      acc_to_smem<BN>(d, img, BN + 4, wg * 64);
-      named_bar(1, 256);
-      epilogue_rows<BN>(p, s.map_c, s.map_z, img, acc, q, lane, s.m_row0, s.n_idx, c_begin, c_end, my_store, s.at,
-                        want_stats ? my_stats : nullptr);
-      if (Work::kSplitK && p.splits > 1) {
-        const Slab t = wk.slab(w, q);
-        splitk_finish_tile(p, t.tile, t.m_idx, t.n_idx, BN, t.c_off, epi_tid, &s_last);
-      }
-      acc ^= 1;
+      const bool res = p.residual != nullptr && p.out_mode != 1;
+      uint4 rv[BN / 16];
+      if (res) res_load<BN>(p, rv, s.m_idx, r0, s.n_idx, lane);
+      if (p.out_mode == 0) {
+        if (lane == 0) tma_store_wait_read<0>();
+        named_bar(1, 256);
+      }
+      if (res) {
+        __syncwarp();
+        res_stage<BN>(rv, stg, r0, lane);
+        __syncwarp();
+      }
+      epilogue_frag<BN>(p, d, stg, wg, s.m_idx, s.n_idx, reinterpret_cast<float*>(s.at.c_ptr ? s.at.c_ptr : p.C));
+      if (p.out_mode == 0) {
+        fence_async_smem();
+        named_bar(1, 256);
+        store_slab<BN>(p, s.map_c, smem_store, q, lane, s.m_row0, s.n_idx, c_begin, c_end, s.at,
+                       want_stats ? my_stats : nullptr);
+      }
+      if (Work::kSplitK && p.splits > 1) splitk_finish_tile(p, s.tile, s.m_idx, s.n_idx, BN, s.c_off, epi_tid, &s_last);
     }
     if (want_stats && stats_n >= 0) stats_flush<BN>(p, s_stats, stats_n, epi_tid);
     if (want_stats) stats_finalize(p, epi_tid);
```
